# nonl4331/raytracing-rust

Hardware: AMD Instinct MI355X
Metric: Msamples/s on rtweekend1.ssml 1920x1080x1024spp (higher is better)
Workload: dtype f32

## Files before the change

### include/rt_hip.h

```cpp
#ifndef RT_HIP_H
#define RT_HIP_H

#include <stdint.h>

#ifdef __cplusplus
extern "C" {
#endif

#define RT_ABI_VERSION 2u

typedef enum rt_status {
	RT_OK = 0,
	RT_ERR_INVALID_ARGUMENT = -1,
	RT_ERR_NO_DEVICE = -2,
	RT_ERR_HIP = -3,
	RT_ERR_OUT_OF_MEMORY = -4,
	RT_ERR_UNSUPPORTED = -5
} rt_status;

typedef enum rt_texture_type {
	RT_TEX_CHECKERED = 0,
	RT_TEX_SOLID = 1,
	RT_TEX_IMAGE = 2,
	RT_TEX_LERP = 3,
// ... 112 lines not shown
	int32_t render_method;
	uint32_t max_depth;
	uint32_t rr_threshold;
	uint32_t shard_index;
	uint32_t shard_count;
	uint32_t tile_width;
	uint32_t tile_height;
	int32_t output_layout;
	uint32_t sample_split;
	uint32_t reserved0;
} rt_render_opts;

void rt_render_opts_default(rt_render_opts *opts);

typedef struct rt_hit_record {
	float t;
	float point[3];
	float error[3];
	float normal[3];
	float uv[2];
	int32_t has_uv;
	int32_t out;
	uint32_t material;
	uint32_t found;
	uint64_t index;
} rt_hit_record;

typedef struct rt_ray_desc {
	float origin[3];
	float direction[3];
} rt_ray_desc;

typedef struct rt_bvh_node {
	float min[3];
	float max[3];
	int64_t children[2];
	uint64_t primitive_offset;
	uint64_t number_primitives;
} rt_bvh_node;

typedef struct rt_scene rt_scene;

const char *rt_last_error(void);
uint32_t rt_abi_version(void);
int rt_device_count(void);

int rt_camera_new(rt_camera *out, const float origin[3], const float lookat[3], const float vup[3],
                  float fov_degrees, float aspect_ratio, float aperture, float focus_dist);

int rt_scene_create(const rt_scene_desc *desc, int device, rt_scene **out);
#define RT_DEVICE_NONE (-1)
void rt_scene_destroy(rt_scene *scene);

int rt_scene_create_multi(const rt_scene_desc *desc, const int *devices, uint32_t n_devices, rt_scene **out);
int rt_scene_device_count(const rt_scene *scene, uint32_t *n_devices);
typedef enum rt_gather_mode { RT_GATHER_NONE = 0, RT_GATHER_RCCL = 1, RT_GATHER_PEER = 2, RT_GATHER_PEER_STAGED = 3, RT_GATHER_SAME_DEVICE = 4 } rt_gather_mode;
int rt_scene_gather_info(const rt_scene *scene, int *mode, char *note, uint64_t note_capacity);
int rt_rccl_probe(int *usable, char *note, uint64_t note_capacity);
int rt_scene_auto_sample_split(const rt_scene *scene, const rt_render_opts *opts, uint32_t *split);

int rt_scene_counts(const rt_scene *scene, uint64_t *n_nodes, uint64_t *n_primitives, uint64_t *n_lights);
int rt_scene_get_nodes(const rt_scene *scene, rt_bvh_node *out, uint64_t capacity);
int rt_scene_get_primitive_order(const rt_scene *scene, uint64_t *out, uint64_t capacity);
int rt_scene_get_lights(const rt_scene *scene, uint64_t *out, uint64_t capacity);
int rt_scene_wide_info(const rt_scene *scene, uint64_t *n_wide_nodes, uint32_t *root_ref, uint32_t *stack_depth);
int rt_scene_get_wide_nodes(const rt_scene *scene, void *out, uint64_t capacity_nodes);
int rt_scene_get_leaf_boxes(const rt_scene *scene, float *out, uint64_t capacity_slots);
int rt_scene_get_wide_nodes_compact(const rt_scene *scene, void *out, uint64_t capacity_nodes);
int rt_scene_get_leaf_boxes_compact(const rt_scene *scene, float *out, uint64_t capacity_leaves, uint64_t *n_leaves);

typedef struct rt_sky_info {
	uint32_t res_x, res_y;
	uint32_t guide_k;
	uint32_t inv_res_ok;
	float inv_res_x, inv_res_y;
	uint64_t table_bytes;
} rt_sky_info;
int rt_scene_sky_info(const rt_scene *scene, rt_sky_info *info);
int rt_scene_get_sky_tables(const rt_scene *scene, float *row_cdf, uint64_t capacity_rows, float *marginal_cdf, uint64_t capacity_marginal,
                            uint8_t *guide, uint64_t capacity_guide);

int rt_scene_set_traversal(rt_scene *scene, int mode);
typedef enum rt_tuning_key { RT_TUNE_TRAVERSAL = 0, RT_TUNE_FEATURE_SET = 1, RT_TUNE_SCENE_IN_LDS = 2, RT_TUNE_SCHEDULE = 3, RT_TUNE_WALK = 4,
                             RT_TUNE_STACK_CAP = 5, RT_TUNE_EXCHANGE = 6, RT_TUNE_WHOLE_PIXEL_SHARE = 7, RT_TUNE_RADIANCE_GROUPS = 8 } rt_tuning_key;
int rt_scene_set_tuning(rt_scene *scene, int key, int value);
int rt_plan_work_items(const rt_render_opts *opts, uint32_t split, int share, uint64_t resident_waves, uint32_t *whole_claims,
                       uint64_t *n_items);

int rt_render(rt_scene *scene, const rt_camera *camera, const rt_render_opts *opts, float *out_rgb,
              uint64_t *rays_shot);

int rt_render_device(rt_scene *scene, const rt_camera *camera, const rt_render_opts *opts, float *d_out_rgb,
                     uint64_t *d_rays_shot, void *hip_stream);

int rt_render_output_floats(const rt_render_opts *opts, uint64_t *n_floats);
int rt_shard_pixel_order(const rt_render_opts *opts, uint64_t *out, uint64_t capacity);

typedef struct rt_sampler_progress {
	uint64_t samples_completed;
	uint64_t rays_shot;
	const float *current_image;
	uint64_t n_floats;
} rt_sampler_progress;
typedef int (*rt_presentation_update)(void *data, const rt_sampler_progress *progress, uint64_t samples_done);
int rt_sample_image(rt_scene *scene, const rt_camera *camera, const rt_render_opts *opts, uint64_t batch,
                    rt_presentation_update update, void *data);

int rt_last_kernel_ms(rt_scene *scene, float *ms, uint32_t *n_launches);

typedef struct rt_launch_info {
	int32_t method;
	int32_t pruned;
	int32_t fine;
	int32_t sky_in_lds;
	int32_t scene_in_lds;
	int32_t feature_set;
	uint32_t block_threads;
	uint32_t n_blocks;
	uint32_t blocks_per_cu;
	uint32_t waves_per_simd;
	uint32_t lds_bytes;
	uint32_t n_cus;
	uint32_t sample_split;
	uint32_t whole_claims;
	uint64_t n_items;
	char kernel[160];
} rt_launch_info;
int rt_last_launch_info(const rt_scene *scene, rt_launch_info *out);

int rt_output_rgb8(const float *rgb, uint64_t n_values, float gamma, uint8_t *out);
int rt_output_save(const char *filename, const float *rgb, uint32_t width, uint32_t height, float gamma);

int rt_output_rgb8_device(rt_scene *scene, const float *d_rgb, uint64_t n_values, float gamma, uint8_t *d_out, void *hip_stream);
int rt_render_rgb8(rt_scene *scene, const rt_camera *camera, const rt_render_opts *opts, float gamma, uint8_t *out_rgb8,
                   uint64_t *rays_shot);

int rt_check_hit(rt_scene *scene, const rt_ray_desc *rays, uint64_t n_rays, rt_hit_record *out);
int rt_check_hit_index(rt_scene *scene, const rt_ray_desc *rays, const uint64_t *object_index, uint64_t n_rays,
                       rt_hit_record *out);

typedef struct rt_radiance_opts {
	uint64_t seed, sample_begin;
	uint32_t samples_per_ray;
	int32_t  render_method;
	uint32_t max_depth;
	uint32_t rr_threshold;
	uint32_t reserved[2];
} rt_radiance_opts;
int rt_radiance_opts_default(rt_radiance_opts *out);
int rt_radiance(rt_scene *scene, const rt_ray_desc *rays, const uint64_t *streams , uint64_t n_rays,
                const rt_radiance_opts *opts, float *out_rgb);
int rt_radiance_device(rt_scene *scene, const rt_ray_desc *d_rays, const uint64_t *d_streams , uint64_t n_rays,
                       const rt_radiance_opts *opts, float *d_out_rgb, void *hip_stream);

typedef struct rt_aov_buffers {
	float *albedo;
	float *normal;
	float *depth;
	float *coverage;
	uint32_t *primitive;
	uint32_t *material;
} rt_aov_buffers;
int rt_render_aov(rt_scene *scene, const rt_camera *camera, const rt_render_opts *opts, const rt_aov_buffers *host_out);
int rt_render_aov_device(rt_scene *scene, const rt_camera *camera, const rt_render_opts *opts, const rt_aov_buffers *device_out,
                         void *hip_stream);

typedef struct rt_aov_chain_opts {
	uint32_t max_chain;
	float fuzz_limit;
	uint32_t reserved[6];
} rt_aov_chain_opts;
typedef struct rt_aov_chain_buffers {
	rt_aov_buffers aov;
	float *bounces;
} rt_aov_chain_buffers;
int rt_aov_chain_opts_default(rt_aov_chain_opts *out);
int rt_render_aov_chain(rt_scene *scene, const rt_camera *camera, const rt_render_opts *opts, const rt_aov_chain_opts *chain,
                        const rt_aov_chain_buffers *host_out);
int rt_render_aov_chain_device(rt_scene *scene, const rt_camera *camera, const rt_render_opts *opts, const rt_aov_chain_opts *chain,
                               const rt_aov_chain_buffers *device_out, void *hip_stream);

#define RT_MATTE_SLOTS 8u
typedef enum { RT_MATTE_ID_PRIMITIVE = 0, RT_MATTE_ID_MATERIAL = 1 } rt_matte_id_kind;
typedef struct rt_matte_opts {
	int32_t id_kind;
	uint32_t layers;
	uint32_t reserved[6];
} rt_matte_opts;
typedef struct rt_matte_buffers {
	uint32_t *ids;
	float *coverage;
	float *residual;
} rt_matte_buffers;
int rt_matte_opts_default(rt_matte_opts *out);
int rt_render_matte(rt_scene *scene, const rt_camera *camera, const rt_render_opts *opts, const rt_matte_opts *matte,
                    const rt_matte_buffers *host_out);
int rt_render_matte_device(rt_scene *scene, const rt_camera *camera, const rt_render_opts *opts, const rt_matte_opts *matte,
                           const rt_matte_buffers *device_out, void *hip_stream);
int rt_matte_extract(rt_scene *scene, const rt_matte_buffers *host_layers, uint32_t width, uint32_t height, uint32_t layers,
                     const uint32_t *ids, uint64_t n_ids, float *host_out);
int rt_matte_extract_device(rt_scene *scene, const rt_matte_buffers *device_layers, uint32_t width, uint32_t height, uint32_t layers,
                            const uint32_t *d_sorted_ids, uint64_t n_ids, float *d_out, void *hip_stream);

typedef struct rt_ao_opts {
	uint32_t rays_per_pass;
	float radius;
	uint32_t reserved[6];
} rt_ao_opts;
typedef struct rt_ao_buffers {
// ... 226 lines not shown
int rt_selftest_division(float divisor, float *reciprocal, int *exact);

#define RT_SELFTEST_LEAN_CLASSES 9
int rt_selftest_lean(int device, uint64_t n_per_thread, uint64_t seed, uint64_t mismatches[RT_SELFTEST_LEAN_CLASSES]);

enum {
	RT_SHORT_FORM_RCP_REFINED = 0,
	RT_SHORT_FORM_INV_ONE_PAIR = 1,
	RT_SHORT_FORM_INV_TWO_PAIRS = 2,
	RT_SHORT_FORM_SQRT_RAW = 3,
	RT_SHORT_FORM_SQRT_BOTH = 4
};
#define RT_SHORT_FORMS 5
enum { RT_SHORT_SITE_RAY_NEW_PAIR = 0, RT_SHORT_SITE_RAY_NEW_FULL = 1 };
#define RT_SHORT_SITES 2
typedef struct rt_short_form_count {
	uint64_t tested;
	uint64_t mismatches;
	uint32_t first_mismatch;
	uint32_t reserved;
} rt_short_form_count;
typedef struct rt_short_forms_result {
	rt_short_form_count form[RT_SHORT_FORMS];
	uint64_t sqrt_raw_exact, sqrt_raw_high, sqrt_raw_low, sqrt_raw_other;
	uint64_t site_tested;
	uint64_t site_mismatches[RT_SHORT_SITES];
	uint32_t in_use;
	uint32_t reserved;
} rt_short_forms_result;
int rt_selftest_short_forms(int device, const float *operands, uint64_t n_operands, rt_short_forms_result *out);

enum { RT_DIV_FORM_ONE_PAIR = 0, RT_DIV_FORM_TWO_PAIRS = 1 };
#define RT_DIV_FORMS 2
enum { RT_DIV_SITE_FIX = 0, RT_DIV_SITE_DIV3_FIX = 1, RT_DIV_SITE_MIS_LIGHT_TERM = 2, RT_DIV_SITE_ATAN2 = 3 };
#define RT_DIV_SITES 4
typedef struct rt_div_forms_slice {
	const uint32_t *denominators;
	uint64_t n_denominators;
	uint32_t first_denominator;
	uint32_t reserved;
	const int32_t *exponents;
	uint64_t n_exponent_pairs;
} rt_div_forms_slice;
typedef struct rt_div_forms_result {
	uint64_t tested;
	uint64_t mismatches[RT_DIV_FORMS];
	uint32_t first_numerator[RT_DIV_FORMS];
	uint32_t first_denominator[RT_DIV_FORMS];
	uint64_t site_tested;
	uint64_t site_in_domain;
	uint64_t site_mismatches[RT_DIV_SITES];
	uint32_t in_use;
	uint32_t reserved;
} rt_div_forms_result;
int rt_selftest_div_forms(int device, const rt_div_forms_slice *slice, const float *operands, uint64_t n_operand_pairs, rt_div_forms_result *out);
int rt_selftest_sky_pdf_forms(rt_scene *scene, const float *dirs, uint64_t m, float *out_pdf_pair, float *out_pdf_default);

enum { RT_FRAME_FORMS_TESTED = 0, RT_FRAME_FORMS_FRAME_MISMATCHES = 1, RT_FRAME_FORMS_FRAME_SHORT = 2, RT_FRAME_FORMS_FRAME_PLAIN = 3,
       RT_FRAME_FORMS_RAY_MISMATCHES = 4, RT_FRAME_FORMS_RAY_SHORT = 5, RT_FRAME_FORMS_RAY_PLAIN = 6, RT_FRAME_FORMS_IN_USE = 7 };
#define RT_FRAME_FORMS_COUNTS 8
enum { RT_FRAME_FORM_FRAME_SHORT = 0, RT_FRAME_FORM_RAY_NORM_ONE_PAIR = 1 };
int rt_selftest_frame_forms(int device, const float *vectors, uint64_t n_vectors, uint64_t counts[RT_FRAME_FORMS_COUNTS]);

enum { RT_GEN_KEYS_TESTED = 0, RT_GEN_KEYS_STATE_MISMATCHES = 1, RT_GEN_KEYS_DRAW_MISMATCHES = 2, RT_GEN_KEYS_ITEM_STATE_MISMATCHES = 3,
       RT_GEN_KEYS_ITEM_DRAW_MISMATCHES = 4, RT_GEN_KEYS_ZERO_BLOCKS = 5, RT_GEN_KEYS_IN_USE = 6 };
#define RT_GEN_KEYS_COUNTS 7
#define RT_GEN_KEYS_CASE_WORDS 4
enum { RT_GEN_KEYS_FORM_TABLE = 0, RT_GEN_KEYS_FORM_ITEM_PRODUCT = 1 };
int rt_selftest_gen_keys(int device, uint64_t seed, const uint32_t *cases, uint64_t n_cases, uint64_t counts[RT_GEN_KEYS_COUNTS]);
void rt_philox_round_keys(uint64_t seed, uint32_t keys[20]);

enum { RT_PAIR_SHADOW_TESTED = 0, RT_PAIR_SHADOW_MISMATCHES = 1, RT_PAIR_SHADOW_ASKED_MISMATCHES = 2, RT_PAIR_SHADOW_ASKED = 3 };
#define RT_PAIR_SHADOW_COUNTS 4
#define RT_PAIR_SHADOW_CASE_FLOATS 10
int rt_selftest_pair_shadow(int device, const float *cases, uint64_t n_cases, uint64_t counts[RT_PAIR_SHADOW_COUNTS]);
enum { RT_PAIR_SHADOW_WALK_TESTED = 0, RT_PAIR_SHADOW_WALK_MISMATCHES = 1, RT_PAIR_SHADOW_WALK_ASKED = 2, RT_PAIR_SHADOW_WALK_ASKED_BOTH = 3,
       RT_PAIR_SHADOW_WALK_ASKED_WITH_OCCLUDED = 4 };
#define RT_PAIR_SHADOW_WALK_COUNTS 5
#define RT_PAIR_SHADOW_WALK_CASE_FLOATS 16
int rt_selftest_pair_shadow_walk(int device, const float *cases, uint64_t n_cases, uint64_t counts[RT_PAIR_SHADOW_WALK_COUNTS]);

int rt_selftest_pair_primary(rt_scene *scene, const float origin[3], uint32_t *valid, uint64_t *mismatches);

int rt_selftest_sky(rt_scene *scene, int tables_in_lds, uint64_t seed, uint64_t n, float *out_dirs, float *out_pdf_of_sample,
                    const float *dirs, uint64_t m, float *out_pdf);

#ifdef __cplusplus
}
#endif
#endif
```

### raytracing-rust_amd/abi.py

```python
import ctypes as C

RT_ABI_VERSION = 2
RT_GATHER_NONE, RT_GATHER_RCCL, RT_GATHER_PEER, RT_GATHER_PEER_STAGED, RT_GATHER_SAME_DEVICE = 0, 1, 2, 3, 4

RT_OK = 0
RT_ERR_INVALID_ARGUMENT = -1
RT_ERR_NO_DEVICE = -2
RT_ERR_HIP = -3
RT_ERR_OUT_OF_MEMORY = -4
RT_ERR_UNSUPPORTED = -5

RT_TEX_CHECKERED, RT_TEX_SOLID, RT_TEX_IMAGE, RT_TEX_LERP, RT_TEX_PERLIN = range(5)
RT_MAT_EMIT, RT_MAT_LAMBERTIAN, RT_MAT_TROWBRIDGE_REITZ, RT_MAT_REFLECT, RT_MAT_REFRACT = range(5)
RT_PRIM_SPHERE, RT_PRIM_TRIANGLE, RT_PRIM_MESH_TRIANGLE = range(3)
RT_SPLIT_SAH, RT_SPLIT_MIDDLE, RT_SPLIT_EQUAL_COUNTS = range(3)
RT_METHOD_NAIVE, RT_METHOD_MIS = range(2)
RT_LAYOUT_FRAME, RT_LAYOUT_SHARD = range(2)
RT_TUNE_TRAVERSAL, RT_TUNE_FEATURE_SET, RT_TUNE_SCENE_IN_LDS, RT_TUNE_SCHEDULE, RT_TUNE_WALK, RT_TUNE_STACK_CAP, RT_TUNE_EXCHANGE, RT_TUNE_WHOLE_PIXEL_SHARE = range(8)
RT_TUNE_RADIANCE_GROUPS = 8

NO_INDEX = 0xFFFFFFFFFFFFFFFF
RT_DEVICE_NONE = -1

f32x3 = C.c_float * 3


class TextureDesc(C.Structure):
    _fields_ = [
        ("type", C.c_int32),
        ("colour_one", f32x3),
        ("colour_two", f32x3),
        ("image_rgb", C.POINTER(C.c_float)),
        ("image_width", C.c_uint32),
        ("image_height", C.c_uint32),
        ("perlin_ran_vecs", C.POINTER(C.c_float)),
        ("perlin_perm", C.POINTER(C.c_uint32)),
    ]


class MaterialDesc(C.Structure):
    _fields_ = [
        ("type", C.c_int32),
        ("texture", C.c_uint32),
        ("param", C.c_float),
        ("ior", f32x3),
        ("metallic", C.c_float),
    ]


class _Sphere(C.Structure):
    _fields_ = [("centre", f32x3), ("radius", C.c_float)]


class _MeshTriangle(C.Structure):
    _fields_ = [("mesh", C.c_uint32), ("point_indices", C.c_uint32 * 3), ("normal_indices", C.c_uint32 * 3)]


class _Triangle(C.Structure):
    _fields_ = [("data", C.c_uint64)]


class _PrimUnion(C.Union):
    _fields_ = [("sphere", _Sphere), ("mesh_triangle", _MeshTriangle), ("triangle", _Triangle)]


class PrimitiveDesc(C.Structure):
    _fields_ = [("type", C.c_int32), ("material", C.c_uint32), ("u", _PrimUnion)]


class TriangleData(C.Structure):
    _fields_ = [("points", C.c_float * 9), ("normals", C.c_float * 9)]


class MeshDesc(C.Structure):
    _fields_ = [
        ("vertices", C.POINTER(C.c_float)),
        ("n_vertices", C.c_uint64),
        ("normals", C.POINTER(C.c_float)),
        ("n_normals", C.c_uint64),
    ]


class SkyDesc(C.Structure):
    _fields_ = [
        ("texture", C.c_uint32),
        ("material", C.c_uint32),
        ("sampler_res_x", C.c_uint32),
        ("sampler_res_y", C.c_uint32),
    ]


class SceneDesc(C.Structure):
    _fields_ = [
        ("abi_version", C.c_uint32),
        ("n_textures", C.c_uint32),
        ("textures", C.POINTER(TextureDesc)),
        ("n_materials", C.c_uint32),
        ("n_meshes", C.c_uint32),
        ("materials", C.POINTER(MaterialDesc)),
        ("meshes", C.POINTER(MeshDesc)),
        ("n_primitives", C.c_uint64),
        ("primitives", C.POINTER(PrimitiveDesc)),
# ... 3 lines not shown
        ("split_type", C.c_int32),
    ]


class Camera(C.Structure):
    _fields_ = [("origin", f32x3), ("lower_left", f32x3), ("horizontal", f32x3), ("vertical", f32x3)]


class RenderOpts(C.Structure):
    _fields_ = [
        ("width", C.c_uint64),
        ("height", C.c_uint64),
        ("samples_per_pixel", C.c_uint64),
        ("sample_begin", C.c_uint64),
        ("seed", C.c_uint64),
        ("render_method", C.c_int32),
        ("max_depth", C.c_uint32),
        ("rr_threshold", C.c_uint32),
        ("shard_index", C.c_uint32),
        ("shard_count", C.c_uint32),
        ("tile_width", C.c_uint32),
        ("tile_height", C.c_uint32),
        ("output_layout", C.c_int32),
        ("sample_split", C.c_uint32),
        ("reserved0", C.c_uint32),
    ]


class HitRecord(C.Structure):
    _fields_ = [
        ("t", C.c_float),
        ("point", f32x3),
        ("error", f32x3),
        ("normal", f32x3),
        ("uv", C.c_float * 2),
        ("has_uv", C.c_int32),
        ("out", C.c_int32),
        ("material", C.c_uint32),
        ("found", C.c_uint32),
        ("index", C.c_uint64),
    ]


class RayDesc(C.Structure):
    _fields_ = [("origin", f32x3), ("direction", f32x3)]


class BvhNode(C.Structure):
    _fields_ = [
        ("min", f32x3),
        ("max", f32x3),
        ("children", C.c_int64 * 2),
        ("primitive_offset", C.c_uint64),
        ("number_primitives", C.c_uint64),
    ]


class SamplerProgressC(C.Structure):
    _fields_ = [
        ("samples_completed", C.c_uint64),
        ("rays_shot", C.c_uint64),
        ("current_image", C.POINTER(C.c_float)),
        ("n_floats", C.c_uint64),
    ]


class LaunchInfo(C.Structure):
    _fields_ = [
        ("method", C.c_int32),
        ("pruned", C.c_int32),
        ("fine", C.c_int32),
        ("sky_in_lds", C.c_int32),
        ("scene_in_lds", C.c_int32),
        ("feature_set", C.c_int32),
        ("block_threads", C.c_uint32),
        ("n_blocks", C.c_uint32),
        ("blocks_per_cu", C.c_uint32),
        ("waves_per_simd", C.c_uint32),
        ("lds_bytes", C.c_uint32),
        ("n_cus", C.c_uint32),
        ("sample_split", C.c_uint32),
        ("whole_claims", C.c_uint32),
        ("n_items", C.c_uint64),
        ("kernel", C.c_char * 160),
    ]


class SkyInfo(C.Structure):
    _fields_ = [
        ("res_x", C.c_uint32),
        ("res_y", C.c_uint32),
        ("guide_k", C.c_uint32),
        ("inv_res_ok", C.c_uint32),
        ("inv_res_x", C.c_float),
        ("inv_res_y", C.c_float),
        ("table_bytes", C.c_uint64),
    ]


class AovBuffers(C.Structure):
    _fields_ = [
        ("albedo", C.POINTER(C.c_float)),
        ("normal", C.POINTER(C.c_float)),
        ("depth", C.POINTER(C.c_float)),
        ("coverage", C.POINTER(C.c_float)),
        ("primitive", C.POINTER(C.c_uint32)),
        ("material", C.POINTER(C.c_uint32)),
    ]


AOV_SHAPES = {"albedo": "hw3", "normal": "hw3", "depth": "hw", "coverage": "hw", "primitive": "hw", "material": "hw"}
AOV_CHANNELS = tuple(AOV_SHAPES)


class AovChainOpts(C.Structure):
    _fields_ = [
        ("max_chain", C.c_uint32),
        ("fuzz_limit", C.c_float),
        ("reserved", C.c_uint32 * 6),
    ]


class AovChainBuffers(C.Structure):
    _fields_ = [
        ("aov", AovBuffers),
        ("bounces", C.POINTER(C.c_float)),
    ]


AOV_CHAIN_SHAPES = {"aov": AOV_SHAPES, "bounces": "hw"}
AOV_CHAIN_CHANNELS = AOV_CHANNELS + ("bounces",)
AOV_CHAIN_MAX_CHAIN = 64


RT_MATTE_SLOTS = 8
RT_MATTE_ID_PRIMITIVE, RT_MATTE_ID_MATERIAL = range(2)
MATTE_ID_KINDS = {"primitive": RT_MATTE_ID_PRIMITIVE, "material": RT_MATTE_ID_MATERIAL}
MATTE_MAX_IDS = 1 << 20


class MatteOpts(C.Structure):
    _fields_ = [
        ("id_kind", C.c_int32),
        ("layers", C.c_uint32),
        ("reserved", C.c_uint32 * 6),
    ]


class MatteBuffers(C.Structure):
    _fields_ = [
        ("ids", C.POINTER(C.c_uint32)),
        ("coverage", C.POINTER(C.c_float)),
        ("residual", C.POINTER(C.c_float)),
    ]


MATTE_SHAPES = {"ids": "lhw", "coverage": "lhw", "residual": "hw"}
MATTE_BUFFERS = tuple(MATTE_SHAPES)


AO_MAX_RAYS = 64


class AoOpts(C.Structure):
    _fields_ = [
        ("rays_per_pass", C.c_uint32),
        ("radius", C.c_float),
# ... 337 lines not shown
    "rt_aov_chain_buffers": (AovChainBuffers, 56),
    "rt_matte_opts": (MatteOpts, 32),
    "rt_matte_buffers": (MatteBuffers, 24),
    "rt_ao_opts": (AoOpts, 32),
    "rt_ao_buffers": (AoBuffers, 16),
    "rt_radiance_opts": (RadianceOpts, 40),
    "rt_noise_opts": (NoiseOpts, 32),
    "rt_noise_summary": (NoiseSummary, 16),
    "rt_noise_buffers": (NoiseBuffers, 40),
    "rt_noise_result": (NoiseResult, 40),
    "rt_adaptive_result": (AdaptiveResult, 40),
    "rt_robust_opts": (RobustOpts, 32),
    "rt_robust_buffers": (RobustBuffers, 40),
    "rt_denoise_opts": (DenoiseOpts, 48),
    "rt_denoise_inputs": (DenoiseInputs, 40),
    "rt_temporal_opts": (TemporalOpts, 96),
    "rt_temporal_inputs": (TemporalInputs, 32),
    "rt_display_opts": (DisplayOpts, 104),
    "rt_display_state": (DisplayState, 16),
    "rt_bloom_opts": (BloomOpts, 64),
    "rt_dof_opts": (DofOpts, 64),
    "rt_upscale_opts": (UpscaleOpts, 56),
    "rt_upscale_inputs": (UpscaleInputs, 56),
    "rt_short_form_count": (ShortFormCount, 24),
    "rt_short_forms_result": (ShortFormsResult, 184),
    "rt_div_forms_slice": (DivFormsSlice, 40),
    "rt_div_forms_result": (DivFormsResult, 96),
}

EXPORTED_SYMBOLS = [
    "rt_last_error",
    "rt_abi_version",
    "rt_device_count",
    "rt_render_opts_default",
    "rt_camera_new",
    "rt_scene_create",
    "rt_scene_create_multi",
    "rt_scene_device_count",
    "rt_scene_destroy",
    "rt_scene_counts",
    "rt_scene_get_nodes",
    "rt_scene_get_primitive_order",
    "rt_scene_get_lights",
    "rt_scene_wide_info",
    "rt_scene_get_wide_nodes",
    "rt_scene_get_leaf_boxes",
    "rt_scene_get_wide_nodes_compact",
    "rt_scene_auto_sample_split",
    "rt_scene_gather_info",
    "rt_rccl_probe",
    "rt_selftest_division",
    "rt_scene_get_leaf_boxes_compact",
    "rt_scene_sky_info",
    "rt_scene_get_sky_tables",
    "rt_scene_set_traversal",
    "rt_scene_set_tuning",
    "rt_render",
    "rt_sample_image",
    "rt_render_device",
    "rt_render_output_floats",
    "rt_shard_pixel_order",
    "rt_plan_work_items",
    "rt_last_kernel_ms",
    "rt_last_launch_info",
    "rt_output_rgb8",
    "rt_output_save",
    "rt_output_rgb8_device",
    "rt_render_rgb8",
    "rt_check_hit",
    "rt_check_hit_index",
    "rt_radiance_opts_default",
    "rt_radiance",
    "rt_radiance_device",
    "rt_selftest_lean",
    "rt_selftest_short_forms",
    "rt_selftest_div_forms",
    "rt_selftest_sky_pdf_forms",
    "rt_selftest_frame_forms",
    "rt_selftest_gen_keys",
    "rt_philox_round_keys",
    "rt_selftest_pair_shadow",
    "rt_selftest_pair_shadow_walk",
    "rt_selftest_pair_primary",
    "rt_selftest_sky",
    "rt_render_aov",
    "rt_render_aov_device",
    "rt_aov_chain_opts_default",
    "rt_render_aov_chain",
    "rt_render_aov_chain_device",
    "rt_matte_opts_default",
    "rt_render_matte",
    "rt_render_matte_device",
    "rt_matte_extract",
    "rt_matte_extract_device",
    "rt_ao_opts_default",
    "rt_render_ao",
    "rt_render_ao_device",
    "rt_denoise_opts_default",
    "rt_denoise_workspace_bytes",
    "rt_denoise",
    "rt_denoise_device",
    "rt_render_denoised",
    "rt_noise_opts_default",
    "rt_render_noise",
    "rt_render_noise_device",
    "rt_noise_tiles",
    "rt_noise_tiles_device",
    "rt_render_converged",
    "rt_render_denoised_split",
    "rt_render_adaptive",
    "rt_render_tiles",
    "rt_render_tiles_device",
    "rt_noise_select_tiles",
    "rt_noise_select_tiles_device",
    "rt_robust_opts_default",
    "rt_render_robust",
    "rt_render_robust_device",
    "rt_robust_combine",
    "rt_robust_combine_device",
    "rt_render_denoised_robust",
    "rt_temporal_opts_default",
    "rt_temporal_history_bytes",
    "rt_temporal_workspace_bytes",
    "rt_denoise_temporal_device",
    "rt_denoise_temporal",
    "rt_denoise_temporal_reset",
    "rt_display_opts_default",
    "rt_display_workspace_bytes",
    "rt_display_output_bytes",
    "rt_display_device",
    "rt_display",
    "rt_display_reset",
    "rt_bloom_opts_default",
    "rt_bloom_workspace_bytes",
    "rt_bloom_device",
    "rt_bloom",
    "rt_dof_opts_default",
    "rt_dof_opts_from_camera",
    "rt_dof_workspace_bytes",
    "rt_dof_device",
    "rt_dof",
    "rt_render_dof",
    "rt_upscale_opts_default",
    "rt_upscale_device",
    "rt_upscale",
    "rt_render_upscaled",
]


def channels(table, struct):
    out = {}
    for name, shape in table.items():
        if isinstance(shape, dict):
            out.update(channels(shape, getattr(struct, name)))
        else:
            out[name] = (struct, dict(struct._fields_)[name]._type_, shape)
    return out


def default_aov_chain_opts(max_chain=8, fuzz_limit=0.0):
    o = AovChainOpts()
    o.max_chain, o.fuzz_limit = max_chain, fuzz_limit
    return o


def default_matte_opts(id_kind=RT_MATTE_ID_MATERIAL, layers=4):
# ... 46 lines not shown
```

### raytracing-rust_amd/csrc/rt_api.cpp

```cpp
#include <hip/hip_runtime.h>

#include <cstdio>
#include <cstdlib>
#include <algorithm>
#include <cmath>
#include <cstring>
#include <string>
#include <vector>

#include "../../include/rt_hip.h"
#include "../../include/rt_detmath.h"
#include <dlfcn.h>
#include "rt_api_internal.h"
#include "rt_render.h"

using namespace rt;

thread_local std::string g_error;

constexpr uint32_t kFineAboveTriangles = 4096;
constexpr uint32_t kFineAboveSpheres = 32768;

struct RcclApi {
	void *lib = nullptr;
// ... 567 lines not shown
		return fail(RT_ERR_INVALID_ARGUMENT, "null argument");
	*mode = s->peers.empty() ? RT_GATHER_NONE : s->gather_mode;
	if (note && note_capacity) {
		std::strncpy(note, s->gather_note.c_str(), (size_t)note_capacity - 1);
		note[note_capacity - 1] = 0;
	}
	return RT_OK;
}

int rt_scene_device_count(const rt_scene *s, uint32_t *n_devices)
{
	if (!s || !n_devices)
		return fail(RT_ERR_INVALID_ARGUMENT, "null argument");
	*n_devices = s->device == RT_DEVICE_NONE ? 0u : (uint32_t)(1 + s->peers.size());
	return RT_OK;
}

int rt_scene_set_traversal(rt_scene *s, int mode)
{
	if (!s || mode < -1 || mode > 1)
		return fail(RT_ERR_INVALID_ARGUMENT, "bad arguments");
	s->traversal_mode = mode;
	for (rt_scene *m : s->peers)
		m->traversal_mode = mode;
	return RT_OK;
}

static int set_tuning_one(rt_scene *s, int key, int value);
int rt_scene_set_tuning(rt_scene *s, int key, int value)
{
	if (!s)
		return fail(RT_ERR_INVALID_ARGUMENT, "null scene");
	const int rc = set_tuning_one(s, key, value);
	for (rt_scene *m : s->peers)
		if (rc == RT_OK) {
			(void)set_tuning_one(m, key, value);
		}
	return rc;
}
static int set_tuning_one(rt_scene *s, int key, int value)
{
	switch (key) {
	case RT_TUNE_TRAVERSAL:
		return rt_scene_set_traversal(s, value);
	case RT_TUNE_FEATURE_SET:
		if (value < s->min_feature_set || value > 2)
			return fail(RT_ERR_INVALID_ARGUMENT, "feature set must be between the scene's own and 2");
		s->feature_set = value;
		s->feature_set_forced = true;
		return RT_OK;
	case RT_TUNE_SCHEDULE:
		if (value < -1 || value > 1)
			return fail(RT_ERR_INVALID_ARGUMENT, "schedule must be -1, 0 or 1");
		s->schedule_mode = value;
		return RT_OK;
	case RT_TUNE_SCENE_IN_LDS:
		s->scene_lds_allowed = value != 0;
		return RT_OK;
	case RT_TUNE_STACK_CAP:
		if (value < 0 || value > 96)
			return fail(RT_ERR_INVALID_ARGUMENT, "stack cap must be 0 (automatic) or 1..96 entries");
		s->stack_cap_override = (uint32_t)value;
		return RT_OK;
	case RT_TUNE_EXCHANGE:
		if (value < 0 || value > 1)
			return fail(RT_ERR_INVALID_ARGUMENT, "exchange must be 0 (off) or 1 (on where the kernel has it)");
		s->exchange_mode = value;
		return RT_OK;
	case RT_TUNE_WHOLE_PIXEL_SHARE:
		if (value < -1 || value > 16)
			return fail(RT_ERR_INVALID_ARGUMENT, "whole-pixel share must be -1 (automatic) or 0..16 (sixteenths of a shard's tiles)");
		s->whole_share = value;
		return RT_OK;
	case RT_TUNE_WALK:
		if (value < 0 || value > 1)
			return fail(RT_ERR_INVALID_ARGUMENT, "walk must be 0 (automatic) or 1 (two-child walk for every ray)");
		s->dev.narrow_only = (uint32_t)value;
		return RT_OK;
	case RT_TUNE_RADIANCE_GROUPS:
		if (value < 0 || value > 65536)
			return fail(RT_ERR_INVALID_ARGUMENT, "radiance groups must be 0 (automatic) or 1..65536 workgroups");
		s->radiance_groups = (uint32_t)value;
		return RT_OK;
	default:
		return fail(RT_ERR_INVALID_ARGUMENT, "unknown tuning key");
	}
}

int rt_scene_counts(const rt_scene *s, uint64_t *n_nodes, uint64_t *n_primitives, uint64_t *n_lights)
{
	if (!s)
		return fail(RT_ERR_INVALID_ARGUMENT, "null scene");
	if (n_nodes) *n_nodes = s->host.nodes.size();
	if (n_primitives) *n_primitives = s->host.primitive_order.size();
	if (n_lights) *n_lights = s->host.lights.size();
	return RT_OK;
}
int rt_scene_get_nodes(const rt_scene *s, rt_bvh_node *out, uint64_t capacity)
{
	if (!s || !out || capacity < s->host.nodes.size())
		return fail(RT_ERR_INVALID_ARGUMENT, "bad arguments");
	for (size_t i = 0; i < s->host.nodes.size(); ++i) {
		const HostNode &n = s->host.nodes[i];
		std::memcpy(out[i].min, n.min, 12);
		std::memcpy(out[i].max, n.max, 12);
		out[i].children[0] = n.child[0];
		out[i].children[1] = n.child[1];
		out[i].primitive_offset = n.primitive_offset;
		out[i].number_primitives = n.number_primitives;
	}
	return RT_OK;
}
int rt_scene_get_primitive_order(const rt_scene *s, uint64_t *out, uint64_t capacity)
{
	if (!s || !out || capacity < s->host.primitive_order.size())
		return fail(RT_ERR_INVALID_ARGUMENT, "bad arguments");
	std::memcpy(out, s->host.primitive_order.data(), s->host.primitive_order.size() * sizeof(uint64_t));
	return RT_OK;
}
int rt_scene_wide_info(const rt_scene *s, uint64_t *n_wide_nodes, uint32_t *root_ref, uint32_t *stack_depth)
{
	if (!s)
		return fail(RT_ERR_INVALID_ARGUMENT, "null scene");
	if (n_wide_nodes) *n_wide_nodes = s->host.dev_nodes4.size();
	if (root_ref) *root_ref = s->host.root4_ref;
	if (stack_depth) *stack_depth = s->host.stack_depth;
	return RT_OK;
}
int rt_scene_get_wide_nodes(const rt_scene *s, void *out, uint64_t capacity_nodes)
{
	if (!s || !out || capacity_nodes < s->host.dev_nodes4.size())
		return fail(RT_ERR_INVALID_ARGUMENT, "bad arguments");
	std::memcpy(out, s->host.dev_nodes4.data(), s->host.dev_nodes4.size() * sizeof(DevNodeQ4));
	return RT_OK;
}
int rt_scene_get_leaf_boxes(const rt_scene *s, float *out, uint64_t capacity_slots)
{
	if (!s || !out || capacity_slots < s->host.leaf_box.size())
		return fail(RT_ERR_INVALID_ARGUMENT, "bad arguments");
	std::memcpy(out, s->host.leaf_box.data(), s->host.leaf_box.size() * sizeof(DevLeafBox));
	return RT_OK;
}
int rt_scene_get_wide_nodes_compact(const rt_scene *s, void *out, uint64_t capacity_nodes)
{
	if (!s || !out || capacity_nodes < s->host.dev_nodes4c.size())
		return fail(RT_ERR_INVALID_ARGUMENT, "bad arguments");
	std::memcpy(out, s->host.dev_nodes4c.data(), s->host.dev_nodes4c.size() * sizeof(DevNodeQ4));
	return RT_OK;
}
int rt_scene_get_leaf_boxes_compact(const rt_scene *s, float *out, uint64_t capacity_leaves, uint64_t *n_leaves)
{
	if (!s)
		return fail(RT_ERR_INVALID_ARGUMENT, "null scene");
	if (n_leaves)
		*n_leaves = s->host.leaf_box_c.size();
	if (!out)
		return n_leaves ? RT_OK : fail(RT_ERR_INVALID_ARGUMENT, "bad arguments");
	if (capacity_leaves < s->host.leaf_box_c.size())
		return fail(RT_ERR_INVALID_ARGUMENT, "bad arguments");
	std::memcpy(out, s->host.leaf_box_c.data(), s->host.leaf_box_c.size() * sizeof(DevLeafBox));
	return RT_OK;
}
int rt_scene_sky_info(const rt_scene *s, rt_sky_info *info)
{
	if (!s || !info)
		return fail(RT_ERR_INVALID_ARGUMENT, "null argument");
// ... 127 lines not shown
	return RT_OK;
}

static void fill_tiling(DevRenderParams &P, const rt_render_opts *o, const ShardGeometry &g)
{
	P.width = (uint32_t)o->width;
	P.height = (uint32_t)o->height;
	P.shard_index = o->shard_index;
	P.shard_count = o->shard_count;
	P.tile_w = g.tile_w;
	P.tile_h = g.tile_h;
	P.tiles_x = g.tiles_x;
	P.tiles_y = g.tiles_y;
	P.n_work = (uint32_t)g.n_work;
}

static uint32_t tiled_order_log2(const rt_render_opts *o, const ShardGeometry &g, uint32_t split)
{
	if (g.tile_w * g.tile_h == 64u && (g.tile_w & (g.tile_w - 1u)) == 0u && o->width < 65536u && o->height < 65536u &&
	    (split & (split - 1u)) == 0u && split <= 64u)
		for (uint32_t lw = 0; lw < 7u; ++lw)
			for (uint32_t ls = 0; ls < 7u; ++ls)
				if ((1u << lw) == g.tile_w && (1u << ls) == split)
					return lw | (ls << 8);
	return 0xFFFFFFFFu;
}

struct RenderLaunchPlan {
	DevRenderParams P;
	DevScene dev;
	bool prune, fine, sky_lds, scene_lds, xchg;
	int feature_set, blocks_per_cu;
	uint32_t block_threads, n_blocks;
	size_t lds_bytes;
	uint32_t split;
};

static int plan_render_launch(const rt_scene *s, const rt_render_opts *o, const ShardGeometry &g, RenderLaunchPlan *plan)
{
	DevRenderParams P;
	std::memset(&P, 0, sizeof P);
	fill_tiling(P, o, g);
	P.spp = (uint32_t)o->samples_per_pixel;
	P.sample_begin_lo = (uint32_t)o->sample_begin;
	P.sample_begin_hi = (uint32_t)(o->sample_begin >> 32);
	P.seed_lo = (uint32_t)o->seed;
	P.seed_hi = (uint32_t)(o->seed >> 32);
	P.max_depth = o->max_depth;
	P.rr_threshold = o->rr_threshold;
	uint32_t split = o->sample_split;
	if (split == 0u)
		split = auto_sample_split(s->n_cus, o->width * o->height, o->samples_per_pixel, o->shard_count);
	{
		float rw = 0.0f, rh = 0.0f;
		const bool sized = o->width <= (1u << 24) && o->height <= (1u << 24);
		const bool ok_w = sized && verified_reciprocal((float)(o->width - 1), &rw), ok_h = sized && verified_reciprocal((float)(o->height - 1), &rh);
		const bool ok = ok_w && ok_h;
		P.w1h1_ok = ok ? 1u : 0u;
		P.inv_w1 = rw;
		P.inv_h1 = rh;
	}
	P.tile_log2_w = tiled_order_log2(o, g, split);
	if (split > o->samples_per_pixel)
		return fail(RT_ERR_INVALID_ARGUMENT, "sample_split larger than samples_per_pixel");
	if (g.n_work * split >= (1ull << 32))
		return fail(RT_ERR_UNSUPPORTED, "pixels x sample_split exceeds 2^32 work items");
	P.sample_split = split;
	P.shard_layout = o->output_layout == RT_LAYOUT_SHARD ? 1 : 0;

	bool prune = scene_prunes(s);
	const bool fine = s->dev.nodes4 != nullptr &&
	                  (s->schedule_mode == -1 ? (prune && s->dev.n_prims > (s->dev.has_triangles ? kFineAboveTriangles : kFineAboveSpheres))
	                                          : s->schedule_mode == 1);
	if (fine)
		prune = true;
	P.prune = prune ? 1 : 0;

	const bool samplable = (s->dev.sky.res_x | s->dev.sky.res_y) != 0u;
	const size_t sky_bytes = sky_table_bytes(s->dev.sky.res_x, s->dev.sky.res_y, s->dev.sky.guide_k);
	const bool scene_lds = !fine && s->dev.blob_bytes != 0u && s->scene_lds_allowed;
	P.scene_in_lds = scene_lds ? 1u : 0u;
	bool sky_lds = false;
	const int feature_set =
	    (s->feature_set == 0 && s->pair_tree && !s->feature_set_forced && !prune && !fine && s->exchange_mode != 1) ? 3 : s->feature_set;
	bool xchg = s->exchange_mode == 1 && render_exchange_available(o->render_method, prune, fine, feature_set);
	const bool xchg_fine = xchg && fine;
	uint32_t block_threads = render_block_threads(feature_set, fine, xchg_fine);
	const size_t fine_pool_bytes = xchg_fine ? render_exchange_fine_lds_bytes(block_threads / 64u) : 0;
	DevScene dev = s->dev;
	const bool walks_wide = prune && dev.nodes4 != nullptr && dev.narrow_only == 0u;
	uint32_t stack_need = (fine || walks_wide) ? dev.stack_depth : s->stack_depth_narrow;
	if (!fine && walks_wide &&
	    render_lds_bytes(dev, false, scene_lds, render_block_threads(feature_set, false, false) / 64u, stack_need) > s->max_lds) {
		dev.narrow_only = 1u;
		stack_need = s->stack_depth_narrow;
	}
	uint32_t stack_cap = stack_need;
	if (fine) {
		const uint32_t blocks_wanted = std::max(1u, render_waves_per_simd(feature_set, true) * 256u / block_threads);
		const size_t share = s->max_lds / blocks_wanted;
		const uint32_t fit = (uint32_t)((share > fine_pool_bytes ? share - fine_pool_bytes : 0) / ((block_threads / 64u) * 64u * 4u));
		stack_cap = std::min(stack_cap, std::max(8u, fit));
	}
	if (fine && s->stack_cap_override != 0u)
		stack_cap = std::min(stack_need, s->stack_cap_override);
	P.stack_cap = stack_cap;
	P.stack_ovf_depth = stack_need - stack_cap;
	const bool sky_lds_possible = samplable && o->render_method == RT_METHOD_MIS && sky_bytes <= kSkyLdsLimit;
	struct Sizing { uint32_t block; int blocks_per_cu; bool sky; size_t lds; };
	auto size_launch = [&](uint32_t block, Sizing &z) -> hipError_t {
		z.block = block;
		z.sky = false;
		z.blocks_per_cu = 0;
		z.lds = render_lds_bytes(dev, false, scene_lds, block / 64u, stack_cap) + fine_pool_bytes;
		if (z.lds > s->max_lds)
			return hipSuccess;
		hipError_t e = render_occupancy(o->render_method, prune, fine, false, feature_set, z.lds, &z.blocks_per_cu, xchg_fine, block);
		if (e != hipSuccess)
			return e;
		if (sky_lds_possible) {
			const size_t lds_with = render_lds_bytes(dev, true, scene_lds, block / 64u, stack_cap) + fine_pool_bytes;
			int blocks_with = 0;
			if (lds_with <= s->max_lds &&
			    render_occupancy(o->render_method, prune, fine, true, feature_set, lds_with, &blocks_with, xchg_fine, block) == hipSuccess &&
			    blocks_with >= z.blocks_per_cu && blocks_with >= 1) {
				z.sky = true;
				z.lds = lds_with;
				z.blocks_per_cu = blocks_with;
			}
		}
		return hipSuccess;
	};
	Sizing Z;
	HIP_TRY(size_launch(block_threads, Z));
	if (Z.lds > s->max_lds)
		return fail(RT_ERR_UNSUPPORTED, "traversal stacks exceed the LDS of one CU");
	if (!fine && !xchg) {
		for (uint32_t cand = block_threads + 256u; cand <= render_max_block_threads(feature_set, fine, false); cand += 256u) {
			Sizing C;
			if (size_launch(cand, C) != hipSuccess || C.blocks_per_cu < 1)
				continue;
			const uint32_t waves_c = (uint32_t)C.blocks_per_cu * C.block, waves_z = (uint32_t)Z.blocks_per_cu * Z.block;
			if (waves_c > waves_z || (waves_c == waves_z && C.sky && !Z.sky))
				Z = C;
		}
		block_threads = Z.block;
	}
	size_t lds_bytes = Z.lds;
	int blocks_per_cu = Z.blocks_per_cu;
	sky_lds = Z.sky;
	P.sky_in_lds = sky_lds ? 1u : 0u;
	if (blocks_per_cu < 1)
		return fail(RT_ERR_HIP, "render kernel does not fit on a CU");
	P.xchg_slots = 0;
	if (xchg && !fine) {
		int blocks_plain = 0;
		if (render_occupancy(o->render_method, prune, fine, sky_lds, feature_set, lds_bytes, &blocks_plain, true) != hipSuccess || blocks_plain < 1) {
			xchg = false;
		} else {
			const int target = std::min(blocks_per_cu, blocks_plain);
			const size_t share = s->max_lds / (size_t)target;
			uint32_t slots = render_exchange_max_slots();
			while (slots >= 16u && lds_bytes + render_exchange_lds_bytes(slots) > share)
				slots -= 4u;
			int blocks_x = 0;
			if (slots >= 16u &&
			    render_occupancy(o->render_method, prune, fine, sky_lds, feature_set, lds_bytes + render_exchange_lds_bytes(slots), &blocks_x, true) == hipSuccess &&
// ... 236 lines not shown
	}
	if (d_rays_shot) {
		for (uint32_t m = 0; m < n; ++m) {
			if (n_floats[m] == 0) {
				HIP_TRY(hipMemsetAsync(head->d_gather_rays + m, 0, sizeof(unsigned long long), stream));
			} else if (members[m]->device == head->device) {
				if (m > 0 && head->gather_mode == RT_GATHER_RCCL)
					HIP_TRY(hipStreamWaitEvent(stream, members[m]->ev_shard, 0));
				HIP_TRY(hipMemcpyAsync(head->d_gather_rays + m, members[m]->d_member_rays, sizeof(unsigned long long), hipMemcpyDeviceToDevice, stream));
			} else {
				if (head->gather_mode == RT_GATHER_RCCL)
					HIP_TRY(hipStreamWaitEvent(stream, members[m]->ev_shard, 0));
				HIP_TRY(hipMemcpyPeerAsync(head->d_gather_rays + m, head->device, members[m]->d_member_rays, members[m]->device, sizeof(unsigned long long), stream));
			}
		}
		HIP_TRY(launch_sum_u64(stream, head->d_gather_rays, n, reinterpret_cast<unsigned long long *>(d_rays_shot)));
	}
	if (!capturing) {
		HIP_TRY(hipEventRecord(head->ev_gathered, stream));
		head->gathered_once = true;
	}
	return RT_OK;
}

int rt_render_device(rt_scene *s, const rt_camera *camera, const rt_render_opts *o, float *d_out_rgb, uint64_t *d_rays_shot,
                     void *hip_stream)
{
	if (!s || !camera || !o || !d_out_rgb)
		return fail(RT_ERR_INVALID_ARGUMENT, "null argument");
	if (!s->peers.empty() && !s->member_call) {
		if (s->device == RT_DEVICE_NONE)
			return fail(RT_ERR_NO_DEVICE, "host-only scene");
		return render_device_multi(s, camera, o, d_out_rgb, d_rays_shot, static_cast<hipStream_t>(hip_stream));
	}
	ShardGeometry g;
	int rc = shard_geometry(o, g);
	if (rc != RT_OK)
		return rc;
	if (s->device == RT_DEVICE_NONE)
		return fail(RT_ERR_NO_DEVICE, "host-only scene (RT_DEVICE_NONE): rendering needs a GPU, there is no CPU fallback");
	if (o->render_method != RT_METHOD_NAIVE && o->render_method != RT_METHOD_MIS)
		return fail(RT_ERR_INVALID_ARGUMENT, "unknown render method");
	if (o->samples_per_pixel == 0 || o->samples_per_pixel >= (1ull << 32))
		return fail(RT_ERR_INVALID_ARGUMENT, "samples_per_pixel must be in [1, 2^32)");
	if (o->output_layout != RT_LAYOUT_FRAME && o->output_layout != RT_LAYOUT_SHARD)
		return fail(RT_ERR_INVALID_ARGUMENT, "unknown output layout");
	HIP_TRY(hipSetDevice(s->device));
	hipStream_t stream = static_cast<hipStream_t>(hip_stream);
	if (g.n_work == 0) {
		HIP_TRY(launch_reset(stream, s->d_work_counter, reinterpret_cast<unsigned long long *>(d_rays_shot), d_out_rgb,
		                     o->output_layout == RT_LAYOUT_FRAME ? (size_t)(o->width * o->height * 3) : 0));
		s->timed = false;
		return RT_OK;
	}

	RenderLaunchPlan plan;
	rc = plan_render_launch(s, o, g, &plan);
	if (rc != RT_OK)
		return rc;
	const DevRenderParams &P = plan.P;
	float *render_target = d_out_rgb;
	if (plan.split > 1u) {
		const size_t need = (size_t)g.n_work * plan.split * 3;
		rc = grow_device_buffer(s->d_partial, s->partial_floats, need);
		if (rc != RT_OK)
			return rc;
		render_target = s->d_partial;
	}
	if (P.stack_ovf_depth != 0u) {
		const size_t need = (size_t)plan.n_blocks * plan.block_threads * P.stack_ovf_depth;
		rc = grow_device_buffer(s->d_stack_ovf, s->stack_ovf_words, need);
		if (rc != RT_OK)
			return rc;
	}
	{
		size_t zero_floats = 0;
		if (o->output_layout == RT_LAYOUT_FRAME && o->shard_count > 1)
			zero_floats = (size_t)(o->width * o->height * 3);
		if (o->output_layout == RT_LAYOUT_SHARD)
			zero_floats = (size_t)(g.n_work * 3);
		HIP_TRY(launch_reset(stream, s->d_work_counter, reinterpret_cast<unsigned long long *>(d_rays_shot), d_out_rgb, zero_floats));
	}
	fill_launch_info(plan, o, s->n_cus, &s->last_launch);
	const DevCamera cam = dev_camera(camera);
	DevPairPrimary primary{};
	if (plan.feature_set == 3)
		pair_primary_terms(s->pair, plan.dev.root_min, plan.dev.root_max, v3(cam.origin[0], cam.origin[1], cam.origin[2]), primary);
	HIP_TRY(hipEventRecord(s->ev_start, stream));
	HIP_TRY(launch_render(o->render_method, plan.prune, plan.fine, plan.sky_lds, plan.feature_set, plan.n_blocks, plan.lds_bytes, stream, plan.dev, cam, P,
	                      render_target, reinterpret_cast<unsigned long long *>(d_rays_shot), s->d_work_counter, s->d_stack_ovf, plan.xchg,
	                      plan.feature_set == 3 ? &s->pair : nullptr, plan.feature_set == 3 ? &primary : nullptr, plan.block_threads));
	HIP_TRY(hipEventRecord(s->ev_stop, stream));
	if (plan.split > 1u)
		HIP_TRY(launch_combine(stream, P, s->d_partial, d_out_rgb));
	s->timed = true;
	s->n_launches = 1;
	return RT_OK;
}

int rt_render(rt_scene *s, const rt_camera *camera, const rt_render_opts *o, float *out_rgb, uint64_t *rays_shot)
{
	if (!s || !camera || !o)
		return fail(RT_ERR_INVALID_ARGUMENT, "null argument");
	if (int rc = need_device(s); rc != RT_OK)
		return rc;
	uint64_t n_floats = 0;
	int rc = rt_render_output_floats(o, &n_floats);
	if (rc != RT_OK)
		return rc;
	if (n_floats == 0) {
		if (rays_shot)
			*rays_shot = 0;
		return RT_OK;
	}
	if (!out_rgb)
		return fail(RT_ERR_INVALID_ARGUMENT, "null argument");
	HIP_TRY(hipSetDevice(s->device));
	rc = ensure_frame_buffers(s, n_floats, false);
	if (rc != RT_OK)
		return rc;
	float *d_out = s->d_prog[0];
	rc = rt_render_device(s, camera, o, d_out, reinterpret_cast<uint64_t *>(s->d_rays), s->stream);
	if (rc != RT_OK)
		return rc;
	Staging st{s};
	st.download(out_rgb, d_out, n_floats * sizeof(float));
	st.download(rays_shot, s->d_rays, sizeof(uint64_t));
	return st.finish("render");
}

int rt_output_rgb8_device(rt_scene *s, const float *d_rgb, uint64_t n_values, float gamma, uint8_t *d_out, void *hip_stream)
{
	if (!s || !d_rgb || !d_out)
		return fail(RT_ERR_INVALID_ARGUMENT, "null argument");
	if (s->device == RT_DEVICE_NONE)
		return fail(RT_ERR_NO_DEVICE, "host-only scene (RT_DEVICE_NONE): this call needs a GPU (rt_output_rgb8 is the host-side conversion)");
	if (n_values == 0)
		return RT_OK;
	HIP_TRY(hipSetDevice(s->device));
	HIP_TRY(launch_quantise(static_cast<hipStream_t>(hip_stream), d_rgb, (size_t)n_values, 1.0f / gamma, d_out));
	return RT_OK;
}

int rt_render_rgb8(rt_scene *s, const rt_camera *camera, const rt_render_opts *o, float gamma, uint8_t *out_rgb8, uint64_t *rays_shot)
{
	if (!s || !camera || !o)
		return fail(RT_ERR_INVALID_ARGUMENT, "null argument");
	if (int rc = need_device(s); rc != RT_OK)
		return rc;
	uint64_t n_values = 0;
	int rc = rt_render_output_floats(o, &n_values);
	if (rc != RT_OK)
		return rc;
	if (n_values == 0) {
		if (rays_shot)
			*rays_shot = 0;
		return RT_OK;
	}
	if (!out_rgb8)
		return fail(RT_ERR_INVALID_ARGUMENT, "null argument");
	HIP_TRY(hipSetDevice(s->device));
	rc = ensure_frame_buffers(s, n_values, false);
	if (rc != RT_OK)
		return rc;
	rc = grow_device_buffer(s->d_rgb8, s->d_rgb8_bytes, (size_t)n_values);
	if (rc != RT_OK)
		return rc;
	float *d_frame = s->d_prog[0];
	rc = rt_render_device(s, camera, o, d_frame, reinterpret_cast<uint64_t *>(s->d_rays), s->stream);
	if (rc != RT_OK)
		return rc;
	Staging st{s};
	st.e = launch_quantise(s->stream, d_frame, (size_t)n_values, 1.0f / gamma, s->d_rgb8);
	st.download(out_rgb8, s->d_rgb8, n_values);
// ... 116 lines not shown
```

### raytracing-rust_amd/csrc/rt_api_internal.h

```cpp
#pragma once
#include <hip/hip_runtime.h>

#include <cstdint>
#include <cstring>
#include <string>
#include <vector>

#include "../../include/rt_hip.h"
#include "rt_build.h"
#include "rt_layout.h"
#include "rt_types.h"

extern thread_local std::string g_error;

inline int fail(int code, const std::string &msg)
{
	g_error = msg;
	return code;
}
inline int hip_fail(hipError_t e, const char *what)
{
	g_error = std::string(what) + ": " + hipGetErrorString(e);
	return e == hipErrorOutOfMemory ? RT_ERR_OUT_OF_MEMORY : RT_ERR_HIP;
}
#define HIP_TRY(expr)                       \
	do {                                    \
		hipError_t e_ = (expr);             \
		if (e_ != hipSuccess)               \
			return hip_fail(e_, #expr);     \
	} while (0)
#define RT_TRY(expr)            \
	do {                        \
		const int rc_ = (expr); \
		if (rc_ != RT_OK)       \
			return rc_;         \
	} while (0)

constexpr uint32_t kPruneAbove = 100;

constexpr int kWholeShareDefault = -1;

struct rt_scene {
	int device = 0;
	rt::HostScene host;
	rt::DevScene dev{};
	std::vector<void *> allocations;
	hipStream_t stream = nullptr;
	uint32_t *d_work_counter = nullptr;
	unsigned long long *d_rays = nullptr;
	hipEvent_t ev_start = nullptr, ev_stop = nullptr;
	bool timed = false;
	uint32_t n_launches = 0;
	int n_cus = 0;
	int traversal_mode = -1;
	int schedule_mode = -1;
	int feature_set = 2;
	int min_feature_set = 0;
	bool pair_tree = false, feature_set_forced = false;
	rt::DevPairScene pair{};
	bool scene_lds_allowed = true;
	float *d_partial = nullptr;
	size_t partial_floats = 0;
	float *d_prog[2] = {nullptr, nullptr};
	float *h_prog[2] = {nullptr, nullptr};
	unsigned long long *d_prog_rays = nullptr;
	unsigned long long *h_prog_rays = nullptr;
	size_t d_prog_floats[2] = {0, 0}, h_prog_floats[2] = {0, 0};
	hipStream_t copy_stream = nullptr;
	hipEvent_t ev_batch[2] = {nullptr, nullptr}, ev_copy[2] = {nullptr, nullptr};
	size_t max_lds = 65536;
	rt_launch_info last_launch{};
	uint32_t stack_cap_override = 0;
	int exchange_mode = 0;
	int whole_share = kWholeShareDefault;
	uint32_t radiance_groups = 0;
	uint32_t stack_depth_narrow = 2;
	uint32_t *d_stack_ovf = nullptr;
	size_t stack_ovf_words = 0;
	uint8_t *d_rgb8 = nullptr;
	size_t d_rgb8_bytes = 0;
	std::vector<rt_scene *> peers;
	bool member_call = false;
	float *d_shard = nullptr;
	size_t shard_floats = 0;
	unsigned long long *d_member_rays = nullptr;
	hipEvent_t ev_shard = nullptr;
	hipEvent_t ev_begin = nullptr;
	float *d_gather = nullptr;
	size_t gather_floats = 0;
	unsigned long long *d_gather_rays = nullptr;
	void *nccl_comms = nullptr;
	int gather_mode = 0;
	std::string gather_note;
	hipEvent_t ev_gathered = nullptr;
	bool gathered_once = false;
	uint32_t *d_prim_desc = nullptr;
	char *d_denoise = nullptr;
	size_t d_denoise_bytes = 0;
	char *d_temporal = nullptr;
	uint32_t temporal_w = 0, temporal_h = 0;
	int temporal_cur = -1;
	rt_camera temporal_prev{};
	char *d_display = nullptr;
	size_t d_display_bytes = 0;
	uint32_t display_w = 0, display_h = 0;
	bool display_has_state = false;
	char *d_noise = nullptr;
	size_t d_noise_bytes = 0;
	char *d_bloom = nullptr;
	size_t d_bloom_bytes = 0;
	char *d_dof = nullptr;
	size_t d_dof_bytes = 0;
};

uint32_t auto_sample_split(int n_cus, uint64_t frame_pixels, uint64_t spp, uint32_t n_sharers);
struct WorkItems { uint64_t whole_claims, n_items; };
WorkItems plan_work_items(uint64_t tiles, uint64_t tile_pixels, uint32_t split, bool tiled, int share, uint64_t resident_waves);

constexpr size_t kSkyLdsLimit = 96 * 1024;
inline size_t sky_table_bytes(uint32_t res_x, uint32_t res_y, uint32_t guide_k)
{
	if ((res_x | res_y) == 0u)
		return 0;
	return ((size_t)res_y * (res_x + 1u) + res_y + 1u) * 4 + (size_t)(res_y + 1u) * guide_k;
}

inline bool scene_prunes(const rt_scene *s)
{
	return s->traversal_mode == -1 ? s->dev.n_prims > kPruneAbove : s->traversal_mode == 1;
}

inline int four_wave_traversal(const rt_scene *s, bool *prune, rt::DevScene *dev)
{
	*prune = scene_prunes(s);
	*dev = s->dev;
	const bool walks_wide = *prune && dev->nodes4 != nullptr && dev->narrow_only == 0u;
	if (!walks_wide || rt::four_wave_stack_lds_bytes(*dev) > s->max_lds) {
		if (walks_wide)
			dev->narrow_only = 1u;
		dev->stack_depth = s->stack_depth_narrow;
	}
	if (rt::four_wave_stack_lds_bytes(*dev) > s->max_lds)
		return fail(RT_ERR_UNSUPPORTED, "traversal stacks exceed the LDS of one CU");
	return RT_OK;
}

inline uint32_t path_lane_groups(const rt_scene *s, size_t lds_bytes, uint32_t waves, uint64_t wanted)
{
	const uint64_t by_lds = std::max<uint64_t>(1, (160u * 1024u) / std::max<size_t>(1, lds_bytes));
	const uint64_t resident = (uint64_t)std::max(1, s->n_cus) * std::min<uint64_t>(waves, by_lds);
	uint64_t groups = std::min<uint64_t>(wanted, resident);
	if (s->radiance_groups != 0u)
		groups = std::min<uint64_t>(groups, s->radiance_groups);
	return (uint32_t)std::max<uint64_t>(groups, 1);
}


struct TileGrid { uint32_t tiles_x; uint64_t count; };
inline TileGrid tile_grid(uint64_t w, uint64_t h)
{
	const uint64_t across = (w + 7) / 8, down = (h + 7) / 8;
	return TileGrid{(uint32_t)across, across * down};
}

struct FrameTiling { uint32_t tile_w, tile_h, tiles_x, tiles_y; uint64_t n_work; };
inline FrameTiling frame_tiling(const rt_render_opts *o)
{
	FrameTiling t;
	t.tile_w = o->tile_width ? o->tile_width : 8;
	t.tile_h = o->tile_height ? o->tile_height : 8;
	t.tiles_x = (uint32_t)((o->width + t.tile_w - 1) / t.tile_w);
	t.tiles_y = (uint32_t)((o->height + t.tile_h - 1) / t.tile_h);
	t.n_work = (uint64_t)t.tiles_x * t.tiles_y * t.tile_w * t.tile_h;
	return t;
}

inline rt::DevCamera dev_camera(const rt_camera *camera)
{
	rt::DevCamera cam;
	std::memcpy(cam.origin, camera->origin, 12);
	std::memcpy(cam.lower_left, camera->lower_left, 12);
	std::memcpy(cam.horizontal, camera->horizontal, 12);
	std::memcpy(cam.vertical, camera->vertical, 12);
	return cam;
}

template <class T> static int upload(rt_scene *s, const T *src, size_t count, const T **dst)
{
	void *p = nullptr;
	const size_t bytes = (count ? count : 1) * sizeof(T);
	HIP_TRY(hipMalloc(&p, bytes));
	s->allocations.push_back(p);
	if (count)
		HIP_TRY(hipMemcpy(p, src, count * sizeof(T), hipMemcpyHostToDevice));
	*dst = static_cast<const T *>(p);
	return RT_OK;
}

inline bool ranges_overlap(const void *a, uint64_t a_bytes, const void *b, uint64_t b_bytes)
{
	if (!a || !b)
		return false;
	const uintptr_t x = reinterpret_cast<uintptr_t>(a), y = reinterpret_cast<uintptr_t>(b);
	return x < y + b_bytes && y < x + a_bytes;
}


inline int need_device(const rt_scene *s)
{
	if (s->device == RT_DEVICE_NONE)
		return fail(RT_ERR_NO_DEVICE, "host-only scene (RT_DEVICE_NONE): this call needs a GPU, there is no CPU fallback");
	return RT_OK;
}

inline int frame_sides(const char *stage, uint64_t w, uint64_t h, uint64_t min_side)
{
	if (w >= min_side && h >= min_side)
		return RT_OK;
	return fail(RT_ERR_INVALID_ARGUMENT, stage + ("width and height must be >= " + std::to_string(min_side)) +
	                                         (min_side >= 2 ? " (u and v divide by W-1 and H-1)" : ""));
}

inline int frame_pixels(const char *stage, uint64_t w, uint64_t h, uint64_t min_side, uint64_t *n)
{
	if (const int rc = frame_sides(stage, w, h, min_side); rc != RT_OK)
		return rc;
	if (w > (1ull << 31) || h > (1ull << 31) || w * h > (1ull << 31))
		return fail(RT_ERR_UNSUPPORTED, std::string(stage) + "more than 2^31 pixels");
	*n = w * h;
	return RT_OK;
}

inline int check_disjoint(const char *message, const void *const buf[], const uint64_t bytes[], int n_written, int n_total)
{
	for (int a = 0; a < n_written; ++a)
		for (int b = 0; b < n_total; ++b)
			if (a != b && ranges_overlap(buf[a], bytes[a], buf[b], bytes[b]))
				return fail(RT_ERR_INVALID_ARGUMENT, message);
	return RT_OK;
}

template <class T> static int grow_device_buffer(T *&p, size_t &count, size_t need)
{
	if (need <= count)
		return RT_OK;
	if (p)
		(void)hipFree(p);
	p = nullptr;
	count = 0;
	HIP_TRY(hipMalloc(reinterpret_cast<void **>(&p), need * sizeof(T)));
	count = need;
	return RT_OK;
}

static int grow_device_buffer(char *&p, size_t &bytes, rt::Layout &L)
{
	if (L.overflowed)
		return fail(RT_ERR_UNSUPPORTED, "internal: a buffer layout of more parts than rt::Layout holds");
	const int rc = grow_device_buffer(p, bytes, (size_t)L.total());
// ... 30 lines not shown
```

### raytracing-rust_amd/csrc/rt_api_query.cpp

```cpp
#include <hip/hip_runtime.h>

#include <algorithm>
#include <cstring>
#include <vector>

#include "../../include/rt_hip.h"
#include "rt_api_internal.h"
#include "rt_query.h"
#include "rt_radiance.h"
#include "rt_selftest.h"
#include "rt_gen_keys.h"

using namespace rt;

#ifdef RT_STATS
extern "C" int rt_debug_trace_queue(rt_scene *s, const rt_ray_desc *rays, uint64_t n, int waves, uint32_t cap, float *out_t, uint32_t *out_prim,
                                    float *ms, unsigned long long *node_steps)
{
	if (!s || !rays || !out_t || !out_prim || n == 0 || n >= (1ull << 31) || s->device == RT_DEVICE_NONE || s->dev.nodes4 == nullptr)
		return fail(RT_ERR_INVALID_ARGUMENT, "bad arguments (or no wide tree)");
	HIP_TRY(hipSetDevice(s->device));
	cap = std::min(std::max(cap, 1u), s->dev.stack_depth);
	const uint32_t ovf_depth = s->dev.stack_depth - cap;
	const uint32_t n_blocks = (uint32_t)s->n_cus * (uint32_t)waves;
// ... 361 lines not shown
	for (int k = 0; k < RT_DIV_SITES; ++k)
		out->site_mismatches[k] = host[kDivCountSiteBad + k];
	out->in_use = div_forms_in_use();
	return RT_OK;
}

int rt_selftest_sky_pdf_forms(rt_scene *s, const float *dirs, uint64_t m, float *out_pdf_pair, float *out_pdf_default)
{
	if (!s || !dirs || !out_pdf_pair || !out_pdf_default || m == 0 || m > (1ull << 24))
		return fail(RT_ERR_INVALID_ARGUMENT, "bad arguments (1 to 2^24 directions)");
	if ((s->host.sky.sampler_res_x | s->host.sky.sampler_res_y) == 0u)
		return fail(RT_ERR_INVALID_ARGUMENT, "the sky is not samplable (sampler_res 0 x 0)");
	if (int rc = need_device(s); rc != RT_OK)
		return rc;
	Layout L;
	const auto p_dirs = L.add<float>(3 * m), p_pair = L.add<float>(m), p_default = L.add<float>(m);
	RT_TRY(sky_buffer(s, L));
	Staging st{s};
	st.put(L, p_dirs, dirs);
	if (st.ok())
		st.e = launch_sky_pdf_forms(s->stream, s->dev, L.at(p_dirs), m, L.at(p_pair), L.at(p_default));
	st.get(out_pdf_pair, L, p_pair);
	st.get(out_pdf_default, L, p_default);
	return sky_finish(st, L, "selftest_sky_pdf_forms");
}

int rt_selftest_pair_shadow(int device, const float *cases, uint64_t n_cases, uint64_t counts[RT_PAIR_SHADOW_COUNTS])
{
	return run_case_table<RT_PAIR_SHADOW_COUNTS>(device, cases, n_cases, RT_PAIR_SHADOW_CASE_FLOATS * sizeof(float), counts, "selftest_pair_shadow",
	                                             launch_pair_shadow);
}
int rt_selftest_pair_shadow_walk(int device, const float *cases, uint64_t n_cases, uint64_t counts[RT_PAIR_SHADOW_WALK_COUNTS])
{
	return run_case_table<RT_PAIR_SHADOW_WALK_COUNTS>(device, cases, n_cases, RT_PAIR_SHADOW_WALK_CASE_FLOATS * sizeof(float), counts,
	                                                  "selftest_pair_shadow_walk", launch_pair_shadow_walk);
}
int rt_selftest_frame_forms(int device, const float *vectors, uint64_t n_vectors, uint64_t counts[RT_FRAME_FORMS_COUNTS])
{
	RT_TRY(run_case_table<RT_FRAME_FORMS_COUNTS>(device, vectors, n_vectors, 3 * sizeof(float), counts, "selftest_frame_forms", launch_frame_forms));
	counts[RT_FRAME_FORMS_IN_USE] = frame_forms_in_use();
	return RT_OK;
}
int rt_selftest_gen_keys(int device, uint64_t seed, const uint32_t *cases, uint64_t n_cases, uint64_t counts[RT_GEN_KEYS_COUNTS])
{
	RT_TRY(run_case_table<RT_GEN_KEYS_COUNTS>(device, cases, n_cases, RT_GEN_KEYS_CASE_WORDS * sizeof(uint32_t), counts, "selftest_gen_keys",
	                                          [seed](hipStream_t stream, const uint32_t *d_cases, uint64_t n, unsigned long long *d_counts) {
		                                          return launch_gen_keys(stream, seed, d_cases, n, d_counts);
	                                          }));
	counts[RT_GEN_KEYS_IN_USE] = gen_keys_in_use();
	return RT_OK;
}

void rt_philox_round_keys(uint64_t seed, uint32_t keys[20])
{
	if (!keys)
		return;
	DevGenKeys K;
	philox_round_keys(seed, K);
	for (int r = 0; r < 10; ++r) {
		keys[2 * r] = K.key[r][0];
		keys[2 * r + 1] = K.key[r][1];
	}
}

int rt_selftest_pair_primary(rt_scene *s, const float origin[3], uint32_t *valid, uint64_t *mismatches)
{
	if (!s || !origin || !valid || !mismatches)
		return fail(RT_ERR_INVALID_ARGUMENT, "null argument");
	if (int rc = need_device(s); rc != RT_OK)
		return rc;
	if (!s->pair_tree)
		return fail(RT_ERR_UNSUPPORTED, "not a scene the two-sphere kernels take");
	DevPairPrimary host{};
	pair_primary_terms(s->pair, s->dev.root_min, s->dev.root_max, v3(origin[0], origin[1], origin[2]), host);
	unsigned long long bad = 0;
	RT_TRY(run_cases(s->device, nullptr, 0, &bad, 1, "selftest_pair_primary", [&](unsigned long long *d, void *) {
		return launch_selftest_pair_primary(nullptr, s->pair, s->dev.root_min, s->dev.root_max, origin, host, d);
	}));
	*valid = host.valid;
	*mismatches = bad;
	return RT_OK;
}

}
```

### raytracing-rust_amd/csrc/rt_intersect.h

```cpp
#pragma once

#include "rt_types.h"
#include "rt_lean.h"

namespace rt {

struct Ray {
	V3 o, d, inv, shear;
};

template <class F> __device__ __forceinline__ Ray ray_new(V3 origin, V3 direction)
{
	Ray r;
	r.o = origin;
#if defined(__HIP_DEVICE_COMPILE__) && !defined(RT_NO_LEAN)
	const float m2 = dot(direction, direction);
	const float smallest = fminf(fminf(fabsf(direction.x), fabsf(direction.y)), fabsf(direction.z));
	if (__builtin_expect(smallest >= 0x1p-60f && m2 >= 0x1p-40f && m2 <= 0x1p40f, 1)) {
		direction = lean_div3_for<lean_ray_norm_short(F::pair)>(direction, lean_sqrt(m2));
		r.d = direction;
		r.inv = v3(lean_inv_for<F::pair>(direction.x), lean_inv_for<F::pair>(direction.y), lean_inv_for<F::pair>(direction.z));
		if (F::tri) {
			const float ax = fabsf(direction.x), ay = fabsf(direction.y), az = fabsf(direction.z);
			const bool swap = (ax > ay && ax > az) || (ay > az);
			const float sx = swap ? direction.z : direction.x;
			const float sz = swap ? direction.x : direction.z;
			const float rz = lean_rcp_refined(sz);
			r.shear = v3(lean_div_core(-sx, sz, rz), lean_div_core(-direction.y, sz, rz), lean_div_core(1.0f, sz, rz));
		} else {
			r.shear = v3s(0.0f);
		}
		return r;
	}
#endif
	direction = direction / mag(direction);
	r.d = direction;
	r.inv = v3(1.0f / direction.x, 1.0f / direction.y, 1.0f / direction.z);
	if (F::tri) {
		const float ax = fabsf(direction.x), ay = fabsf(direction.y), az = fabsf(direction.z);
		const bool swap = (ax > ay && ax > az) || (ay > az);
		const float sx = swap ? direction.z : direction.x;
		const float sz = swap ? direction.x : direction.z;
		r.shear = v3(-sx / sz, -direction.y / sz, 1.0f / sz);
	} else {
		r.shear = v3s(0.0f);
	}
	return r;
}
__device__ __forceinline__ bool ray_swaps_xz(const Ray &r)
{
	const float ax = fabsf(r.d.x), ay = fabsf(r.d.y), az = fabsf(r.d.z);
	return (ax > ay && ax > az) || (ay > az);
}

template <class D> __device__ __forceinline__ bool aabb_slabs(const D &delta, const V3 &inv, float &tmin_out)
{
	constexpr float widen = 1.0f + 2.0f * gamma_n(3);
	float t1 = delta(0, false) * inv.x;
	float t2 = delta(0, true) * inv.x;
	if (t1 > t2) { const float s = t1; t1 = t2; t2 = s; }
	t2 *= widen;
	float tmin = fmin_(t1, t2);
	float tmax = fmax_(t1, t2);

	t1 = delta(1, false) * inv.y;
	t2 = delta(1, true) * inv.y;
	if (t1 > t2) { const float s = t1; t1 = t2; t2 = s; }
	t2 *= widen;
	tmin = fmax_(tmin, fmin_(t1, t2));
	tmax = fmin_(tmax, fmax_(t1, t2));

	t1 = delta(2, false) * inv.z;
	t2 = delta(2, true) * inv.z;
	if (t1 > t2) { const float s = t1; t1 = t2; t2 = s; }
	t2 *= widen;
	tmin = fmax_(tmin, fmin_(t1, t2));
	tmax = fmin_(tmax, fmax_(t1, t2));

	tmin_out = tmin;
	return tmax > fmax_(tmin, 0.0f);
}
__device__ __forceinline__ bool aabb_does_int(const float bmin[3], const float bmax[3], const Ray &r, float &tmin_out)
{
	const float o[3] = {r.o.x, r.o.y, r.o.z};
	return aabb_slabs([&](int axis, bool upper) { return (upper ? bmax[axis] : bmin[axis]) - o[axis]; }, r.inv, tmin_out);
}
__device__ __forceinline__ bool aabb_does_int_from(const float dmin[3], const float dmax[3], const V3 &inv, float &tmin_out)
{
	return aabb_slabs([&](int axis, bool upper) { return upper ? dmax[axis] : dmin[axis]; }, inv, tmin_out);
}

__device__ __forceinline__ float sqrt_from_(float x)
{
// ... 806 lines not shown
```

### raytracing-rust_amd/csrc/rt_render.h

```cpp
#pragma once
#include <hip/hip_runtime.h>
#include "rt_types.h"

namespace rt {
size_t render_lds_bytes(const DevScene &S, bool sky_lds, bool scene_lds, uint32_t waves_per_block, uint32_t stack_cap);
uint32_t render_waves_per_simd(int feature_set, bool fine);
uint32_t render_block_threads(int feature_set, bool fine, bool xchg = false);
uint32_t render_max_block_threads(int feature_set, bool fine, bool xchg);
hipError_t render_occupancy(int method, bool prune, bool fine, bool sky_lds, int feature_set, size_t lds_bytes, int *blocks_per_cu, bool xchg,
                            uint32_t block_threads = 0);
bool render_exchange_available(int method, bool prune, bool fine, int feature_set);
size_t render_exchange_lds_bytes(uint32_t slots);
uint32_t render_exchange_max_slots();
size_t render_exchange_fine_lds_bytes(uint32_t waves_per_block);

hipError_t launch_reset(hipStream_t stream, uint32_t *work_counter, unsigned long long *rays_shot, float *out, size_t n_out_floats);
hipError_t launch_render(int method, bool prune, bool fine, bool sky_lds, int feature_set, uint32_t n_blocks, size_t lds_bytes, hipStream_t stream,
                         const DevScene &S, const DevCamera &cam, const DevRenderParams &P, float *out,
                         unsigned long long *rays_shot, uint32_t *work_counter, uint32_t *stack_ovf, bool xchg, const DevPairScene *pair,
                         const DevPairPrimary *primary, uint32_t block_threads = 0);
hipError_t launch_combine(hipStream_t stream, const DevRenderParams &P, const float *partial, float *out);
hipError_t launch_scatter_shard(hipStream_t stream, const DevRenderParams &P, const float *shard, float *frame);
hipError_t launch_sum_u64(hipStream_t stream, const unsigned long long *parts, uint32_t n, unsigned long long *out);
hipError_t launch_quantise(hipStream_t stream, const float *rgb, size_t n_values, float inv_gamma, uint8_t *out);
}
```

### raytracing-rust_amd/csrc/rt_render.hip

```cpp
#include "rt_shade.h"
#include "rt_gen_keys.h"
#include "rt_render.h"

namespace rt {

enum : int {
	PH_GEN = 0,
	PH_NODE = 1,
	PH_LEAF = 2,
	PH_SHADE = 3,
	PH_LIGHT = 4,
	PH_SCATTER = 5,
	PH_NARROW = 6,
	PH_COUNT = 7,
	PH_NEED_PIXEL = 7,
	PH_DONE = 8,
	PH_WALK = 9
};

#ifndef RT_PQ_SPLIT
#define RT_PQ_SPLIT 1
#endif
#ifndef RT_LIGHT_PHASE_THRESHOLD
#define RT_LIGHT_PHASE_THRESHOLD 48
#endif
constexpr uint32_t kLightPhaseThreshold = RT_LIGHT_PHASE_THRESHOLD;
#ifndef RT_STARVE_LIMIT
#define RT_STARVE_LIMIT 128
#endif
constexpr uint32_t kStarveLimit = RT_STARVE_LIMIT;
constexpr uint32_t kClaim = 64;
constexpr uint32_t kWholePixel = 64u;
constexpr uint32_t kWholeClaim = 1u << 31;
#ifndef RT_ACQUIRE_BATCH
#define RT_ACQUIRE_BATCH 1
#endif
constexpr uint32_t kAcquireBatch = RT_ACQUIRE_BATCH;
#ifndef RT_FULL_WAVES
#define RT_FULL_WAVES 5
#endif
#ifndef RT_FULL_FINE_WAVES
#define RT_FULL_FINE_WAVES 4
#endif
#ifndef RT_SIMPLE_FINE_WAVES
#define RT_SIMPLE_FINE_WAVES 4
#endif
#ifndef RT_SIMPLE_COARSE_WAVES
#define RT_SIMPLE_COARSE_WAVES 5
#endif
#ifndef RT_SIMPLE_COARSE_BLOCK
#define RT_SIMPLE_COARSE_BLOCK 256
#endif
#ifndef RT_SPHERES_BLOCK
#define RT_SPHERES_BLOCK 512
#endif
#ifndef RT_FUSE_REGIONS
#define RT_FUSE_REGIONS(spheres_only) true
#endif
#ifndef RT_BODY_ALWAYS
#define RT_BODY_ALWAYS(spheres_only) true
#endif
#ifndef RT_SPHERES_MAX_BLOCK
#define RT_SPHERES_MAX_BLOCK 768
#endif
#ifndef RT_PAIR_WAVES
#define RT_PAIR_WAVES 6
#endif
#ifndef RT_SPHERES_WAVES
#define RT_SPHERES_WAVES 4
#endif
#ifndef RT_SPHERES_COARSE_WAVES
#define RT_SPHERES_COARSE_WAVES 6
#endif

__device__ __forceinline__ float power_heuristic(float pdf_a, float pdf_b)
{
	const float a_sq = pdf_a * pdf_a;
	return a_sq / (a_sq + pdf_b * pdf_b);
}

__device__ __forceinline__ bool work_to_pixel(const DevRenderParams &P, uint32_t w, uint32_t &x, uint32_t &y)
{
	const uint32_t tile_pixels = P.tile_w * P.tile_h;
	const uint32_t k = w / tile_pixels;
	const uint32_t in = w - k * tile_pixels;
	const uint32_t tile = P.shard_index + k * P.shard_count;
	const uint32_t ty = tile / P.tiles_x;
	const uint32_t tx = tile - ty * P.tiles_x;
	x = tx * P.tile_w + in % P.tile_w;
	y = ty * P.tile_h + in / P.tile_w;
	return x < P.width && y < P.height;
}

template <class F, bool FINE = false, bool XCHG = false> struct KernelShape {
	static constexpr bool spheres_only = !(F::tri || F::lights || F::cmat || F::ctex);
	static constexpr bool simple = !spheres_only && !(F::cmat || F::ctex);
	static constexpr int waves_per_simd = (F::cmat || F::ctex) ? (FINE ? RT_FULL_FINE_WAVES : (XCHG ? 3 : RT_FULL_WAVES))
	                                      : (F::pair ? RT_PAIR_WAVES : (spheres_only ? ((FINE || XCHG) ? RT_SPHERES_WAVES : RT_SPHERES_COARSE_WAVES)
	                                                                                 : (FINE ? RT_SIMPLE_FINE_WAVES : (XCHG ? 4 : RT_SIMPLE_COARSE_WAVES))));
	static constexpr int block = (FINE && XCHG) ? 512 : (spheres_only ? RT_SPHERES_BLOCK : ((simple && !FINE) ? RT_SIMPLE_COARSE_BLOCK : 256));
	static constexpr int max_block = ((spheres_only || simple) && !FINE && !XCHG && block == 512) ? RT_SPHERES_MAX_BLOCK : block;
};

#ifdef RT_STATS
#define RT_SECTION(k) do { const unsigned long long now_ = wall_clock64(); st_sect[(k)] += now_ - st_mark; st_mark = now_; } while (0)
#else
#define RT_SECTION(k) do { } while (0)
#endif
#ifdef RT_STATS
__device__ unsigned long long g_stats[64];
__device__ unsigned long long g_hist[4][65];
#endif

constexpr uint32_t kXchgBStride = 44, kXchgPStride = 12;
constexpr uint32_t kXchgMaxSlots = 64;
constexpr uint32_t kXchgMinLanes = 4;
constexpr uint32_t kXchgRecWords = 60;
constexpr uint32_t kXchgFineSlots = 64;
constexpr uint32_t kXchgFineHdr = 8 + 2 * 64;
#ifndef RT_XCHG_SHADERS
#define RT_XCHG_SHADERS 1
#endif
constexpr uint32_t kXchgShaderWaves = RT_XCHG_SHADERS;
enum : uint32_t { XS_EMPTY = 0, XS_FULL = 1, XS_BUSY = 2 };

struct RenderArgs {
	DevScene S;
	DevCamera cam;
	DevRenderParams P;
	float *out;
	unsigned long long *rays_shot;
	uint32_t *work_counter;
	uint32_t *stack_ovf;
	DevPairScene pair;
	DevPairPrimary primary;
	DevGenKeys gen_keys;
};
#if defined(__HIP_DEVICE_COMPILE__)
typedef const __attribute__((address_space(4))) RenderArgs *KArgs;
#else
typedef const RenderArgs *KArgs;
#endif

template <int METHOD, bool PRUNE, bool FINE, bool SKY_LDS, class F, bool XCHG = false>
__global__ __launch_bounds__((KernelShape<F, FINE, XCHG>::max_block), (KernelShape<F, FINE, XCHG>::waves_per_simd)) void render_kernel(const RenderArgs args_by_value)
{
	extern __shared__ __align__(16) uint32_t lds[];
	const uint32_t lane = threadIdx.x & 63u;
	const uint32_t wave = threadIdx.x >> 6;

	(void)args_by_value;
#if defined(__HIP_DEVICE_COMPILE__)
	const KArgs K = (KArgs)__builtin_amdgcn_kernarg_segment_ptr();
	auto kargs = [&]() -> KArgs {
		KArgs k = K;
		asm volatile("" : "+s"(k));
		return k;
	};
#else
	const KArgs K = &args_by_value;
	auto kargs = [&]() -> KArgs { return K; };
#endif
	DevPairScene PS = {};
	auto load_pair_boxes = [&]() {
		if constexpr (F::pair) {
			const KArgs k = kargs();
#pragma unroll
			for (int i = 0; i < 3; ++i) {
				PS.c0min[i] = k->pair.c0min[i]; PS.c0max[i] = k->pair.c0max[i];
				PS.c1min[i] = k->pair.c1min[i]; PS.c1max[i] = k->pair.c1max[i];
			}
		}
	};
	auto load_pair_scene = [&](auto with_boxes) {
		if constexpr (F::pair) {
			if constexpr (decltype(with_boxes)::value)
				load_pair_boxes();
			const KArgs k = kargs();
#pragma unroll
			for (int i = 0; i < 3; ++i) {
				PS.sky_c1[i] = k->pair.sky_c1[i]; PS.sky_c2[i] = k->pair.sky_c2[i];
			}
			PS.slot0 = k->pair.slot0; PS.slot1 = k->pair.slot1; PS.rank0 = k->pair.rank0; PS.rank1 = k->pair.rank1;
#pragma unroll
			for (int i = 0; i < 4; ++i) {
				PS.sphere[0][i] = k->pair.sphere[0][i]; PS.sphere[1][i] = k->pair.sphere[1][i];
				PS.lambert[0][i] = k->pair.lambert[0][i]; PS.lambert[1][i] = k->pair.lambert[1][i];
			}
			PS.inv_radius[0] = k->pair.inv_radius[0]; PS.inv_radius[1] = k->pair.inv_radius[1];
			PS.sky_param = k->pair.sky_param;
			PS.sky_tex_type = k->pair.sky_tex_type;
		}
	};
	DevPairPrimary PP = {};
	auto load_pair_primary = [&]() {
		if constexpr (F::pair) {
			const KArgs k = kargs();
#pragma unroll
			for (int i = 0; i < 3; ++i) {
				PP.box[0][0][i] = k->primary.box[0][0][i]; PP.box[0][1][i] = k->primary.box[0][1][i];
				PP.box[1][0][i] = k->primary.box[1][0][i]; PP.box[1][1][i] = k->primary.box[1][1][i];
			}
#pragma unroll
			for (int i = 0; i < 4; ++i) {
				PP.sphere[0][i] = k->primary.sphere[0][i]; PP.sphere[1][i] = k->primary.sphere[1][i];
			}
			PP.valid = k->primary.valid;
		}
	};
	const DevScene S_global = K->S;
	const DevRenderParams P = K->P;
	uint32_t *const stack_ovf = K->stack_ovf;
	DevScene S = S_global;

	SkyTables T;
	uint32_t sky_words = 0;
	if (SKY_LDS) {
		const uint32_t n_rows = S.sky.res_y * (S.sky.res_x + 1u);
		const uint32_t n_all = n_rows + S.sky.res_y + 1u;
		float *lds_sky = reinterpret_cast<float *>(lds);
		for (uint32_t i = threadIdx.x; i < n_all; i += blockDim.x)
			lds_sky[i] = S.sky.row_cdf[i];
		__syncthreads();
		sky_words = (n_all + 3u) & ~3u;
		const uint32_t guide_words = (S.sky.res_y + 1u) * S.sky.guide_k / 4u;
		uint32_t *lds_guide = lds + sky_words;
		const uint32_t *src_guide = reinterpret_cast<const uint32_t *>(S.sky.guide);
		for (uint32_t i = threadIdx.x; i < guide_words; i += blockDim.x)
			lds_guide[i] = src_guide[i];
		__syncthreads();
		T.row_cdf = lds_sky;
		T.marginal_cdf = lds_sky + n_rows;
		T.guide = reinterpret_cast<const uint8_t *>(lds_guide);
		sky_words += guide_words;
	} else {
		T.row_cdf = S.sky.row_cdf;
		T.marginal_cdf = S.sky.marginal_cdf;
		T.guide = S.sky.guide;
	}
	T.guide_k = S.sky.guide_k;
	T.inv_res = reinterpret_cast<KWords>(&K->S.sky.inv_res_ok);
	uint32_t blob_words = 0;
	if (!FINE && P.scene_in_lds) {
		uint32_t *lds_blob = lds + sky_words;
		blob_words = S.blob_bytes / 4u;
		for (uint32_t i = threadIdx.x; i < blob_words; i += blockDim.x)
			lds_blob[i] = S.blob[i];
		__syncthreads();
		const char *b = reinterpret_cast<const char *>(lds_blob);
		S.nodes = reinterpret_cast<const DevNode *>(b + S.off_nodes);
		S.prims = reinterpret_cast<const DevPrim *>(b + S.off_prims);
		S.shade = reinterpret_cast<const DevShade *>(b + S.off_shade);
		S.prim_rank = reinterpret_cast<const uint32_t *>(b + S.off_rank);
		S.materials = reinterpret_cast<const DevMaterial *>(b + S.off_materials);
		S.textures = reinterpret_cast<const DevTexture *>(b + S.off_textures);
		S.lights = reinterpret_cast<const uint32_t *>(b + S.off_lights);
		S.big_leaves = reinterpret_cast<const uint2 *>(b + S.off_big_leaves);
	}
	StackMem SM;
	SM.cap = P.stack_cap;
	SM.ovf_depth = P.stack_ovf_depth;
	SM.ovf = stack_ovf;
	SM.region = lds + sky_words + blob_words;
	uint32_t *stk = SM.region + wave * (P.stack_cap * kStackStride) + lane;
	uint32_t *pool = nullptr;
	if constexpr (XCHG) {
		pool = lds + (((uint32_t)(SM.region - lds) + (blockDim.x >> 6) * (P.stack_cap * kStackStride) + 3u) & ~3u);
		if (FINE) {
			if (threadIdx.x < kXchgFineHdr)
				pool[threadIdx.x] = threadIdx.x == 3u ? kXchgShaderWaves : (threadIdx.x == 4u ? (blockDim.x >> 6) - kXchgShaderWaves : 0u);
		} else if (threadIdx.x < 4u) {
			pool[threadIdx.x] = 0u;
		}
		__syncthreads();
	}

#ifdef RT_STATS
	unsigned long long st_iters[2] = {0, 0}, st_active[2] = {0, 0}, st_gen = 0, st_hist[8] = {};
	unsigned long long st_sect[16] = {}, st_mark = wall_clock64();
	unsigned long long st_fine_clock[PH_COUNT + 1] = {};
	unsigned long long st_fine_iters[PH_COUNT] = {}, st_fine_active[PH_COUNT] = {};
#endif
	const bool sky_samplable = sky_can_sample(S);
	constexpr bool kWholeItems = F::pair && !FINE;
	static_assert(!(kWholeItems && XCHG), "the exchange's records carry chunk_begin and chunk_end, not chunk_c: no whole-pixel items there");
	constexpr int known_path = F::known_materials ? kMatLambertian : kMatRead;
	constexpr bool kKeyedGen = kWholeItems && lean_gen_keys(F::pair);
	constexpr bool kItemProduct = kWholeItems && lean_gen_item_product(F::pair);

	int ph = PH_NEED_PIXEL;
	rt_rng rng = {1u, 2u, 3u, 4u};
	Ray ray;
	ray.o = ray.d = ray.inv = ray.shear = v3s(0.0f);
	uint32_t node = kRefDone;
	int sp = 0;
	float best_t = 0.0f;
	uint32_t best_prim = kNoPrim;
	bool any_hit = false;
	V3 thr = v3s(1.0f), outp = v3s(0.0f), mean = v3s(0.0f), wo = v3s(0.0f);
	Hit hit;
	hit.t = 0.0f;
	hit.point = hit.error = hit.normal = v3s(0.0f);
	hit.err_dot = 0.0f;
	hit.uvx = hit.uvy = 0.0f;
	hit.has_uv = hit.out = false;
	uint32_t mat = 0;
	uint32_t depth = 0, out_index = 0, pixel_index = 0, px = 0, py = 0;
	uint32_t sample_i = 0, chunk_begin = 0, chunk_end = P.spp, chunk_c = 0;
	uint32_t ray_count = 0;
	unsigned long long rays_total = 0;
	bool primary = true;
	uint32_t gen_hi0 = 0, gen_lo0 = 0;
	struct LightCtx {
		V3 l_wi;
		float pdf_multiplier;
		float t_limit;
		uint32_t skip;
		bool have_shadow, shadow_is_sky;
	};
	LightCtx PL;
	PL.l_wi = v3s(0.0f);
	PL.pdf_multiplier = 1.0f;
	PL.t_limit = 0.0f;
	PL.skip = kNoPrim;
	PL.have_shadow = PL.shadow_is_sky = false;

	auto begin_walk = [&](bool shadow) {
		any_hit = shadow;
		best_t = 0.0f;
		best_prim = kNoPrim;
		sp = 0;
		if (!FINE) {
			ph = PH_NODE;
			return;
		}
		if (XCHG) {
			ph = PH_WALK;
			return;
		}
		if (root_box_misses(S, ray)) {
			node = kRefDone;
			ph = shadow ? PH_SCATTER : PH_SHADE;
		} else if (S.narrow_only != 0u || !ray_is_regular(ray)) {
			ph = PH_NARROW;
		} else {
			node = S.root4_ref;
			ph = ref_is_leaf(node) ? PH_LEAF : PH_NODE;
		}
	};
	auto start_walk = [&]() {
		sp = 0;
		if (root_box_misses(S, ray)) {
			node = kRefDone;
			ph = any_hit ? PH_SCATTER : PH_SHADE;
		} else if (S.narrow_only != 0u || !ray_is_regular(ray)) {
			ph = PH_NARROW;
		} else {
			node = S.root4_ref;
			ph = ref_is_leaf(node) ? PH_LEAF : PH_NODE;
		}
	};
	auto after_step = [&]() {
		if (node == kRefDone)
			ph = any_hit ? PH_SCATTER : PH_SHADE;
		else
			ph = ref_is_leaf(node) ? PH_LEAF : PH_NODE;
	};
	auto finalize = [&](bool filter) {
		V3 c = outp;
		if (filter && (contains_nan(c) || !is_finite_any(c)))
			c = v3s(0.0f);
		if (P.sample_split > 1u) {
			mean.x += c.x;
			mean.y += c.y;
			mean.z += c.z;
		} else {
			const float i_f = (float)(sample_i + 1u);
			mean.x += (c.x - mean.x) / i_f;
			mean.y += (c.y - mean.y) / i_f;
			mean.z += (c.z - mean.z) / i_f;
		}
		rays_total += ray_count;
		sample_i += 1;
		if (sample_i == chunk_end) {
			const KArgs k = kargs();
			float *const out = k->out;
			out[3u * (size_t)out_index + 0u] = mean.x;
			out[3u * (size_t)out_index + 1u] = mean.y;
			out[3u * (size_t)out_index + 2u] = mean.z;
			ph = PH_NEED_PIXEL;
			if constexpr (kWholeItems) {
				const uint32_t log2_s = k->P.tile_log2_w >> 8;
				const uint32_t c1 = (chunk_c & (kWholePixel - 1u)) + 1u;
				if (chunk_c >= kWholePixel && (c1 >> log2_s) == 0u) {
					chunk_c += 1u;
					chunk_end = (uint32_t)(((uint64_t)(c1 + 1u) * k->P.spp) >> log2_s);
					out_index += k->P.n_work;
					mean = v3s(0.0f);
					ph = PH_GEN;
				}
			}
		} else {
			ph = PH_GEN;
		}
	};

	auto do_gen = [&]() {
		const KArgs k = kargs();
		const uint64_t seed = ((uint64_t)k->P.seed_hi << 32) | k->P.seed_lo;
		const uint64_t sample_begin = ((uint64_t)k->P.sample_begin_hi << 32) | k->P.sample_begin_lo;
		const V3 cam_o = v3(k->cam.origin[0], k->cam.origin[1], k->cam.origin[2]);
		const V3 cam_ll = v3(k->cam.lower_left[0], k->cam.lower_left[1], k->cam.lower_left[2]);
		const V3 cam_h = v3(k->cam.horizontal[0], k->cam.horizontal[1], k->cam.horizontal[2]);
		const V3 cam_v = v3(k->cam.vertical[0], k->cam.vertical[1], k->cam.vertical[2]);
		const uint32_t w1 = here_(k->P.width - 1u), h1 = here_(k->P.height - 1u);
		if constexpr (kKeyedGen) {
			uint32_t hi0 = gen_hi0, lo0 = gen_lo0;
			if constexpr (!kItemProduct)
				philox_pixel_product(pixel_index, hi0, lo0);
			rng_seed_keyed<lean_gen_keys_lead(F::pair)>(&rng, &k->gen_keys, hi0, lo0, sample_begin + chunk_begin + sample_i);
		} else {
			rt_rng_seed(&rng, seed, (uint64_t)pixel_index, sample_begin + chunk_begin + sample_i);
		}
		RT_SECTION(15);
		const float jx = rt_rng_range_f32(&rng, 0.0f, 1.0f) + (float)px, jy = rt_rng_range_f32(&rng, 0.0f, 1.0f) + (float)py;
		float u, v;
		if (here_(k->P.w1h1_ok) != 0u) {
			u = div_by_verified(jx, (float)w1, k->P.inv_w1);
			v = 1.0f - div_by_verified(jy, (float)h1, k->P.inv_h1);
		} else {
			u = div_tame_fix_(jx, (float)w1);
			v = 1.0f - div_tame_fix_(jy, (float)h1);
		}
		ray = ray_new<F>(cam_o, cam_ll + cam_h * u + cam_v * v - cam_o);
		(void)rt_rng_f32(&rng);
		thr = v3s(1.0f);
		outp = v3s(0.0f);
		depth = 0;
		ray_count = 0;
		primary = true;
		begin_walk(false);
	
	};

#ifdef RT_STATS
	unsigned long long st_lane_nodes = 0, st_lane_prims = 0, st_lane_maxsp = 0;
#endif
	auto do_node = [&]() {
#ifdef RT_STATS
		st_lane_nodes += 1;
		if ((unsigned long long)sp > st_lane_maxsp)
			st_lane_maxsp = (unsigned long long)sp;
#endif
		const bool limit_valid = any_hit ? !(PL.t_limit != PL.t_limit) : (best_prim != kNoPrim);
		if (SM.ovf_depth == 0u)
			node = descend4<PRUNE, false>(S, SM, ray, node, stk, sp, limit_valid, any_hit ? PL.t_limit : best_t);
		else
			node = descend4<PRUNE, true>(S, SM, ray, node, stk, sp, limit_valid, any_hit ? PL.t_limit : best_t);
		after_step();
	
	};

	auto do_leaf = [&]() {
		uint32_t first, count, leaf_ref;
		const bool candidate = wide_leaf_hit(S, node, ray, leaf_ref);
		leaf_range(S, leaf_ref, first, count);
		if (!candidate)
			count = 0u;
		bool occluded = false;
		for (uint32_t slot = first; slot < first + count; ++slot) {
			if (any_hit && slot == PL.skip)
				continue;
#ifdef RT_STATS
			st_lane_prims += 1;
#endif
			const PrimGeom g = load_prim<F>(S, slot);
			float t;
			if (prim_t<F>(g, ray, t) && t > 0.0f) {
				if (any_hit) {
					if (!(t >= PL.t_limit)) {
						occluded = true;
						break;
					}
				} else {
					bool take;
					if (best_prim == kNoPrim)
						take = true;
					else if (t < best_t)
						take = true;
					else if (t == best_t)
						take = S.prim_rank[slot] < S.prim_rank[best_prim];
					else
						take = false;
					if (take) {
						best_t = t;
						best_prim = slot;
					}
				}
			}
		}
		if (occluded) {
			best_prim = 0u;
			node = kRefDone;
		} else if (sp == 0) {
			node = kRefDone;
		} else {
			--sp;
			node = SM.ovf_depth == 0u ? stack_load<false>(SM, stk, sp) : stack_load<true>(SM, stk, sp);
		}
		after_step();
	
	};

	auto do_shade = [&](auto arm_tag) {
		constexpr int arm = decltype(arm_tag)::value;
		const uint32_t prim = best_prim;
		bool finish = false;
		bool filter = true;
		Hit nh;
		uint32_t nmat;
		if (prim != kNoPrim)
			make_hit<F>(S, prim, ray, best_t, nh, nmat, PS);
		else
			make_sky_hit_lean<F>(S, nh, nmat);
		const int known_new = F::known_materials ? (prim == kNoPrim ? kMatEmit : kMatLambertian) : kMatRead;

		if (METHOD == 0) {
			ray_count += 1;
			const V3 wo_n = ray.d;
// ... 490 lines not shown
		const bool is_e = (mE >> lane & 1ull) != 0ull;
		if (!will_bounce) {
			uint32_t can = nb >= kXchgMinLanes ? min(nb, slots - cB) : 0u;
			if (!fresh)
				can = min(can, cP);
			if (ph == PH_LIGHT && rB < can) {
				park_path(cB + rB);
				if (rB < cP)
					take_pixel(cP - 1u - rB);
				else
					ph = PH_NEED_PIXEL;
			}
			cB += can;
			cP -= min(can, cP);
			const uint32_t te = min(ne, cP);
			if (is_e && rE < te)
				take_pixel(cP - 1u - rE);
			cP -= te;
		} else {
			const uint32_t swaps = np >= kXchgMinLanes ? min(min(np, cB), slots - cP) : 0u;
			if (ph == PH_GEN && rP < swaps) {
				park_pixel(cP + rP);
				take_path(cB - 1u - rP);
			}
			cB -= swaps;
			cP += swaps;
			const uint32_t te = min(ne, cB);
			if (is_e && rE < te)
				take_path(cB - 1u - rE);
			cB -= te;
			if (nb == 0u && np == 0u && te == 0u) {
				const uint32_t tp = min(ne, cP);
				if (is_e && rE < tp)
					take_pixel(cP - 1u - rE);
				cP -= tp;
			}
		}
		__builtin_amdgcn_fence(__ATOMIC_RELEASE, "workgroup");
		if (lane == 0u) {
			pool[1] = cB;
			pool[2] = cP;
			__hip_atomic_store(&pool[0], 0u, __ATOMIC_RELEASE, __HIP_MEMORY_SCOPE_WORKGROUP);
		}
	};

	uint32_t wq_next = 0, wq_end = 0;
	uint32_t wq_xy = 0, wq_pbase = 0;
	auto acquire_coarse = [&]() {
		const unsigned long long need = __ballot(ph == PH_NEED_PIXEL);
		if (kAcquireBatch > 1u && (uint32_t)__popcll(need) < kAcquireBatch && __ballot(ph == PH_GEN || ph == PH_LIGHT) != 0ull)
			return;
		const KArgs k = kargs();
		const bool tiled = P.tile_log2_w != 0xFFFFFFFFu;
		uint32_t avail = 0, old_next = 0, old_xy = 0, old_pbase = 0, base = 0, log2_w = 0, log2_s = 0;
		if (need != 0ull) {
			const uint32_t n = (uint32_t)__popcll(need);
#if defined(RT_STATS) && !defined(RT_STATS_NO_HIST)
			if (lane == 0u)
				atomicAdd(&g_hist[2][n], 1ull);
#endif
			avail = wq_end - wq_next;
			old_next = wq_next, old_xy = wq_xy, old_pbase = wq_pbase;
			if (tiled)
				log2_w = k->P.tile_log2_w & 7u, log2_s = k->P.tile_log2_w >> 8;
			base = wq_end;
			if (avail < n) {
				const int leader = __ffsll((long long)need) - 1;
				uint32_t claimed = 0;
				if ((int)lane == leader)
					claimed = atomicAdd(k->work_counter, kClaim);
				base = (uint32_t)__builtin_amdgcn_readlane((int)claimed, leader);
				if (tiled) {
					const uint32_t b = base >> 6;
					const uint32_t whole = kWholeItems ? k->P.whole_claims : 0u;
					const bool is_whole = b < whole;
					const uint32_t bc = is_whole ? 0u : b - whole;
					const uint32_t kt = is_whole ? b : whole + (bc >> log2_s);
					const uint32_t sub = bc & ((1u << log2_s) - 1u);
					const uint32_t tile = k->P.shard_index + kt * k->P.shard_count;
					const uint32_t ty = tile / k->P.tiles_x;
					const uint32_t tx = tile - ty * k->P.tiles_x;
					wq_xy = (tx << log2_w) | ((ty * k->P.tile_h) << 16);
					wq_pbase = ((kt << 6) + (sub << (6u - log2_s))) | (is_whole ? kWholeClaim : 0u);
				}
				wq_next = base + (n - avail);
				wq_end = base + kClaim;
			} else {
				wq_next += n;
			}
		}
		if (ph == PH_NEED_PIXEL) {
			const uint32_t r = (uint32_t)__popcll(need & ((1ull << lane) - 1ull));
			const bool from_old = r < avail;
			const uint32_t w = from_old ? old_next + r : base + (r - avail);
			const uint32_t spp = k->P.spp;
			bool inside;
			if (tiled) {
				const uint32_t xy = from_old ? old_xy : wq_xy;
				const uint32_t in = w & 63u;
				const uint32_t pbase = from_old ? old_pbase : wq_pbase;
				const bool whole = kWholeItems && pbase >= kWholeClaim;
				const uint32_t ls = whole ? 0u : log2_s;
				const uint32_t wp = (kWholeItems ? pbase & (kWholeClaim - 1u) : pbase) + (in >> ls);
				const uint32_t c = in & ((1u << ls) - 1u);
				const uint32_t in_tile = wp & 63u;
				px = (xy & 0xFFFFu) + (in_tile & ((1u << log2_w) - 1u));
				py = (xy >> 16) + (in_tile >> log2_w);
				inside = px < k->P.width && py < k->P.height;
				pixel_index = py * k->P.width + px;
				const uint32_t first = (uint32_t)(((uint64_t)c * spp) >> log2_s);
				const uint32_t end = (uint32_t)(((uint64_t)(c + 1u) * spp) >> log2_s);
				if constexpr (kWholeItems) {
					sample_i = first;
					chunk_end = end;
					chunk_c = c | (whole ? kWholePixel : 0u);
				} else {
					chunk_begin = first;
					chunk_end = end - first;
				}
				out_index = log2_s != 0u ? c * k->P.n_work + wp : (k->P.shard_layout ? wp : pixel_index);
			} else {
				const uint32_t split = k->P.sample_split, n_work = k->P.n_work;
				inside = work_to_pixel(P, split > 1u ? w % n_work : w, px, py);
				pixel_index = py * k->P.width + px;
				if constexpr (kWholeItems)
					chunk_c = 0u;
				if (split > 1u) {
					const uint32_t c = w / n_work;
					const uint32_t first = (uint32_t)(((uint64_t)c * spp) / split);
					const uint32_t end = (uint32_t)(((uint64_t)(c + 1u) * spp) / split);
					if constexpr (kWholeItems) {
						sample_i = first;
						chunk_end = end;
					} else {
						chunk_begin = first;
						chunk_end = end - first;
					}
					out_index = w;
				} else {
					if constexpr (kWholeItems)
						sample_i = 0u;
					else
						chunk_begin = 0u;
					chunk_end = spp;
					out_index = k->P.shard_layout ? w : pixel_index;
				}
			}
			if constexpr (kItemProduct)
				philox_pixel_product(pixel_index, gen_hi0, gen_lo0);
			if (w >= k->P.n_items) {
				ph = PH_DONE;
			} else if (inside) {
				if constexpr (!kWholeItems)
					sample_i = 0;
				mean = v3s(0.0f);
				ph = PH_GEN;
			}
		}
	};
	auto acquire = [&]() {
	if constexpr (!FINE) {
		acquire_coarse();
		return;
	}
	{
		const unsigned long long need = __ballot(ph == PH_NEED_PIXEL);
		if (need != 0ull) {
			const KArgs k = kargs();
			const DevRenderParams P = k->P;
			const uint32_t n = (uint32_t)__popcll(need);
			const uint32_t avail = wq_end - wq_next;
			uint32_t base = wq_end;
			if (avail < n) {
				const int leader = __ffsll((long long)need) - 1;
				uint32_t claimed = 0;
				if ((int)lane == leader)
					claimed = atomicAdd(k->work_counter, kClaim);
				base = __shfl(claimed, leader);
			}
			if (ph == PH_NEED_PIXEL) {
				const uint32_t r = (uint32_t)__popcll(need & ((1ull << lane) - 1ull));
				const uint32_t w = r < avail ? wq_next + r : base + (r - avail);
				if (w >= P.n_items) {
					ph = PH_DONE;
				} else if (work_to_pixel(P, P.sample_split > 1u ? w % P.n_work : w, px, py)) {
					pixel_index = py * P.width + px;
					if (P.sample_split > 1u) {
						const uint32_t c = w / P.n_work;
						chunk_begin = (uint32_t)(((uint64_t)c * P.spp) / P.sample_split);
						chunk_end = (uint32_t)(((uint64_t)(c + 1u) * P.spp) / P.sample_split) - chunk_begin;
						out_index = w;
					} else {
						out_index = P.shard_layout ? w : pixel_index;
					}
					sample_i = 0;
					mean = v3s(0.0f);
					ph = PH_GEN;
				}
// ... 29 lines not shown
				if (k != PH_NODE && run < 0 && cnt[k] >= (k == PH_NARROW ? 1u : (k == PH_LEAF ? kDrainLanes : kDrainLanesHeavy))) {
					run = k;
					best_n = cnt[k];
				}
			}
			if (run < 0 && cnt[PH_NODE] > 0u && !(XCHG && xchg_shader)) {
				run = PH_NODE;
				best_n = cnt[PH_NODE];
			}
			if (run < 0) {
#pragma unroll
				for (int k = 0; k < PH_COUNT; ++k) {
					if (cnt[k] >= best_n && cnt[k] > 0u) {
						best_n = cnt[k];
						run = k;
					}
				}
			}
			if (run < 0) {
				if (XCHG && __ballot(ph == PH_WALK) != 0ull) {
					__builtin_amdgcn_s_sleep(4);
					continue;
				}
				if (__ballot(ph == PH_NEED_PIXEL) == 0ull) {
					if (XCHG && !xchg_try_exit()) {
						__builtin_amdgcn_s_sleep(4);
						continue;
					}
					break;
				}
				continue;
			}
#ifdef RT_STATS
			if (lane == 0u) {
				st_fine_iters[run] += 1;
				st_fine_active[run] += best_n;
			}
#endif
#ifdef RT_STATS
			if (lane == 0u) {
				const unsigned long long now_ = wall_clock64();
				st_fine_clock[PH_COUNT] += now_ - st_mark;
				st_mark = now_;
			}
#endif
			if (run == PH_NODE) {
#pragma unroll 1
				for (int step = 0; step < kNodeStepsPerVote; ++step)
					if (ph == PH_NODE)
						do_node();
			} else if (run == PH_LEAF) {
				if (ph == PH_LEAF)
					do_leaf();
			} else if (run == PH_GEN) {
				if (ph == PH_GEN)
					do_gen();
			} else if (run == PH_SHADE) {
				if (ph == PH_SHADE)
					do_shade(std::integral_constant<int, 0>{});
			} else if (run == PH_LIGHT) {
				if (ph == PH_LIGHT)
					do_light(PL, ray);
			} else if (run == PH_NARROW) {
				if (ph == PH_NARROW)
					do_narrow();
			} else {
				if (ph == PH_SCATTER)
					do_scatter(PL, ray);
			}
#ifdef RT_STATS
			if (lane == 0u) {
				const unsigned long long now_ = wall_clock64();
				st_fine_clock[run] += now_ - st_mark;
				st_mark = now_;
			}
#endif
		}
	}

	if constexpr (!FINE) {
		bool alive = true;
		uint32_t waited = 0;
		while (alive) {
			if (XCHG && METHOD == 1)
				exchange();
			acquire();
			const uint32_t n_light = (uint32_t)__popcll(__ballot(ph == PH_LIGHT));
			const uint32_t n_trace = (METHOD == 1 && RT_PQ_SPLIT) ? (uint32_t)__popcll(__ballot(ph == PH_GEN))
			                                                      : (uint32_t)__popcll(__ballot(ph == PH_GEN || ph == PH_NODE || ph == PH_LEAF || ph == PH_SHADE));
			constexpr bool kBodyAlways = RT_BODY_ALWAYS(KernelShape<F>::spheres_only);
			if (kBodyAlways) {
				alive = (n_light + n_trace != 0u) || __ballot(ph == PH_NEED_PIXEL) != 0ull;
				if (XCHG && METHOD == 1 && !alive)
					alive = __hip_atomic_load(&pool[1], __ATOMIC_RELAXED, __HIP_MEMORY_SCOPE_WORKGROUP) != 0u ||
					        __hip_atomic_load(&pool[2], __ATOMIC_RELAXED, __HIP_MEMORY_SCOPE_WORKGROUP) != 0u;
			}
			if (kBodyAlways || n_light + n_trace != 0u) {
				const bool run_light = (METHOD == 1) && (n_light >= kLightPhaseThreshold || n_trace == 0u || (kStarveLimit != 0u && waited >= kStarveLimit));
				waited = run_light ? 0u : waited + n_light;
	#ifdef RT_STATS
				if (lane == 0u) {
					if (!run_light) {
						st_iters[0] += 1; st_active[0] += n_trace;
						st_hist[((n_trace ? n_trace : 1u) - 1u) >> 3] += 1;
#ifndef RT_STATS_NO_HIST
						atomicAdd(&g_hist[0][n_trace], 1ull);
						atomicAdd(&g_hist[1][n_light], 1ull);
#endif
						st_gen += (unsigned long long)__popcll(__ballot(ph == PH_GEN));
					} else {
						st_iters[1] += 1; st_active[1] += n_light;
#ifndef RT_STATS_NO_HIST
						atomicAdd(&g_hist[3][n_light], 1ull);
#endif
					}
				}
	#endif
				RT_SECTION(0);
				constexpr bool kFuseRegions = METHOD == 1 && RT_PQ_SPLIT && RT_FUSE_REGIONS(KernelShape<F>::spheres_only);
				bool run_q = run_light;
				if (!run_light) {
					if (kFuseRegions) {
						if (ph == PH_GEN) {
							load_pair_scene(std::false_type{});
							do_gen();
							load_pair_primary();
							RT_SECTION(1);
							walk_closest_primary();
							RT_SECTION(2);
							do_shade(std::integral_constant<int, 1>{});
						}
						RT_SECTION(3);
						const uint32_t n_light_now = (uint32_t)__popcll(__ballot(ph == PH_LIGHT));
						run_q = n_light_now >= kLightPhaseThreshold;
						if (run_q)
							waited = 0u;
	#ifdef RT_STATS
						if (run_q && lane == 0u) {
							st_iters[1] += 1; st_active[1] += n_light_now;
						}
	#endif
					} else {
						load_pair_scene(std::true_type{});
						if (ph == PH_GEN)
							do_gen();
						RT_SECTION(1);
						walk_closest_pending();
						RT_SECTION(2);
						if (ph == PH_SHADE)
							do_shade(std::integral_constant<int, (METHOD == 1 && RT_PQ_SPLIT) ? 1 : 0>{});
						RT_SECTION(3);
					}
				}
				if (run_q) {
					LightCtx L;
					L.l_wi = v3s(0.0f);
					L.pdf_multiplier = 1.0f;
					L.t_limit = 0.0f;
					L.skip = kNoPrim;
					L.have_shadow = L.shadow_is_sky = false;
					Ray sray;
					sray.o = sray.d = sray.inv = sray.shear = v3s(0.0f);
					if (kFuseRegions) {
						if (ph == PH_LIGHT) {
							load_pair_scene(std::true_type{});
							do_light(L, sray);
							RT_SECTION(4);
							walk_shadow_pending(L, sray);
							RT_SECTION(5);
							do_scatter(L, sray);
							RT_SECTION(6);
							if (ph == PH_NODE) {
								walk_closest_pending();
								RT_SECTION(7);
								do_shade(std::integral_constant<int, 2>{});
							}
						}
						RT_SECTION(8);
					} else {
						load_pair_scene(std::true_type{});
						if (ph == PH_LIGHT)
							do_light(L, sray);
						RT_SECTION(4);
						walk_shadow_pending(L, sray);
						RT_SECTION(5);
						if (ph == PH_SCATTER)
							do_scatter(L, sray);
						RT_SECTION(6);
	#if RT_PQ_SPLIT
						walk_closest_pending();
						RT_SECTION(7);
						if (ph == PH_SHADE)
							do_shade(std::integral_constant<int, 2>{});
						RT_SECTION(8);
	#endif
					}
				}
	#if RT_PQ_SPLIT
				if (METHOD == 1) {
					ray.o = ray.d = ray.inv = ray.shear = v3s(0.0f);
					best_t = 0.0f;
					best_prim = kNoPrim;
					node = kRefDone;
					sp = 0;
					any_hit = false;
				}
	#endif
			} else {
				alive = __ballot(ph == PH_NEED_PIXEL) != 0ull;
				if (XCHG && METHOD == 1)
					alive = alive || __hip_atomic_load(&pool[1], __ATOMIC_RELAXED, __HIP_MEMORY_SCOPE_WORKGROUP) != 0u ||
					        __hip_atomic_load(&pool[2], __ATOMIC_RELAXED, __HIP_MEMORY_SCOPE_WORKGROUP) != 0u;
			}
		}
	}
#ifdef RT_STATS
	atomicAdd(&g_stats[20], st_lane_nodes);
	atomicAdd(&g_stats[21], st_lane_prims);
	atomicMax(&g_stats[22], st_lane_maxsp);
	if (lane == 0u) {
		for (int k = 0; k < 9; ++k)
			atomicAdd(&g_stats[40 + k], st_sect[k]);
		if (!FINE)
			for (int k = 9; k < 16; ++k)
				atomicAdd(&g_stats[40 + k], st_sect[k]);
		for (int k = 0; k < 8; ++k)
			atomicAdd(&g_stats[24 + k], st_hist[k]);
		for (int k = 0; k <= PH_COUNT; ++k)
			atomicAdd(&g_stats[50 + k], st_fine_clock[k]);
		atomicAdd(&g_stats[0], st_iters[0]); atomicAdd(&g_stats[1], st_active[0]);
		atomicAdd(&g_stats[2], st_iters[1]); atomicAdd(&g_stats[3], st_active[1]);
		atomicAdd(&g_stats[4], st_gen);
		for (int k = 0; k < PH_COUNT; ++k) {
			atomicAdd(&g_stats[5 + k], st_fine_iters[k]);
			atomicAdd(&g_stats[5 + PH_COUNT + k], st_fine_active[k]);
		}
	}
#endif
	unsigned long long *const rays_shot = K->rays_shot;
	if (rays_shot != nullptr) {
		for (int off = 32; off > 0; off >>= 1)
			rays_total += __shfl_down(rays_total, off);
		if (lane == 0u)
			atomicAdd(rays_shot, rays_total);
	}
}

__global__ __launch_bounds__(256) void combine_chunks_kernel(const DevRenderParams P, const float *__restrict__ partial, float *__restrict__ out)
{
	const uint32_t wp = blockIdx.x * blockDim.x + threadIdx.x;
	if (wp >= P.n_work)
		return;
	uint32_t x, y;
	if (!work_to_pixel(P, wp, x, y))
		return;
	V3 acc = v3s(0.0f);
	for (uint32_t c = 0; c < P.sample_split; ++c) {
		const float *m = partial + 3u * ((size_t)c * P.n_work + wp);
		acc.x = acc.x + m[0];
		acc.y = acc.y + m[1];
		acc.z = acc.z + m[2];
	}
	const size_t o = P.shard_layout ? (size_t)wp : (size_t)y * P.width + x;
	out[3u * o + 0u] = acc.x / (float)P.spp;
	out[3u * o + 1u] = acc.y / (float)P.spp;
	out[3u * o + 2u] = acc.z / (float)P.spp;
}

__global__ __launch_bounds__(256) void reset_kernel(uint32_t *__restrict__ work_counter, unsigned long long *__restrict__ rays_shot,
                                                    float *__restrict__ out, size_t n_out_floats)
{
	const size_t i = (size_t)blockIdx.x * blockDim.x + threadIdx.x;
	if (i == 0) {
		*work_counter = 0u;
		if (rays_shot)
			*rays_shot = 0ull;
	}
	for (size_t k = i; k < n_out_floats; k += (size_t)gridDim.x * blockDim.x)
		out[k] = 0.0f;
}
hipError_t launch_reset(hipStream_t stream, uint32_t *work_counter, unsigned long long *rays_shot, float *out, size_t n_out_floats)
{
	size_t blocks = (n_out_floats + 255) / 256;
	if (blocks < 1)
		blocks = 1;
	if (blocks > 4096)
		blocks = 4096;
	hipLaunchKernelGGL(reset_kernel, dim3((uint32_t)blocks), dim3(256), 0, stream, work_counter, rays_shot, out, n_out_floats);
	return hipGetLastError();
}

__global__ __launch_bounds__(256) void quantise_kernel(const float *__restrict__ rgb, size_t n_values, float inv_gamma, uint8_t *__restrict__ out)
{
	const size_t stride = (size_t)gridDim.x * blockDim.x;
	const size_t n4 = n_values / 4;
	for (size_t i = (size_t)blockIdx.x * blockDim.x + threadIdx.x; i < n4; i += stride) {
		const float4 v = reinterpret_cast<const float4 *>(rgb)[i];
		const uint32_t q = (uint32_t)rt_quantise_u8(v.x, inv_gamma) | ((uint32_t)rt_quantise_u8(v.y, inv_gamma) << 8) |
		                   ((uint32_t)rt_quantise_u8(v.z, inv_gamma) << 16) | ((uint32_t)rt_quantise_u8(v.w, inv_gamma) << 24);
		reinterpret_cast<uint32_t *>(out)[i] = q;
	}
	if (blockIdx.x == 0 && threadIdx.x < (n_values & 3))
		out[n4 * 4 + threadIdx.x] = rt_quantise_u8(rgb[n4 * 4 + threadIdx.x], inv_gamma);
}
__global__ __launch_bounds__(256) void quantise_unaligned_kernel(const float *__restrict__ rgb, size_t n_values, float inv_gamma, uint8_t *__restrict__ out)
{
	const size_t stride = (size_t)gridDim.x * blockDim.x;
	for (size_t i = (size_t)blockIdx.x * blockDim.x + threadIdx.x; i < n_values; i += stride)
		out[i] = rt_quantise_u8(rgb[i], inv_gamma);
}
hipError_t launch_quantise(hipStream_t stream, const float *rgb, size_t n_values, float inv_gamma, uint8_t *out)
{
	if ((reinterpret_cast<uintptr_t>(rgb) & 15u) != 0u || (reinterpret_cast<uintptr_t>(out) & 3u) != 0u) {
		size_t blocks = (n_values + 255) / 256;
		blocks = blocks < 1 ? 1 : (blocks > 16384 ? 16384 : blocks);
// ... 124 lines not shown
using FeatSimple = Feat<true, true, false, false>;

template <class F> static render_fn pick_render_f(int method, bool prune, bool fine, bool sky_lds, bool xchg)
{
#ifdef RT_ONLY_HEADLINE
	if constexpr (!(F::cmat || F::ctex))
		if (method == 1 && !prune && !fine && sky_lds && !xchg)
			return render_kernel<1, false, false, true, F>;
#ifdef RT_HEADLINE_RUNNABLE
	if constexpr (!(F::cmat || F::ctex))
		if (method == 1 && !prune && !fine && !sky_lds && !xchg)
			return render_kernel<1, false, false, false, F>;
#endif
	return nullptr;
#else
	if constexpr (F::pair) {
		if (xchg || prune || fine)
			return nullptr;
		if (method == 0)
			return render_kernel<0, false, false, false, F>;
		return sky_lds ? render_kernel<1, false, false, true, F> : render_kernel<1, false, false, false, F>;
	} else {
	if (xchg) {
		if (method == 1 && !prune && !fine)
			return sky_lds ? render_kernel<1, false, false, true, F, true> : render_kernel<1, false, false, false, F, true>;
		if (fine && method == 0)
			return render_kernel<0, true, true, false, F, true>;
		if (fine && method == 1)
			return sky_lds ? render_kernel<1, true, true, true, F, true> : render_kernel<1, true, true, false, F, true>;
		return nullptr;
	}
#define RT_PICK(M, P, G, L) \
	if (method == M && prune == P && fine == G && sky_lds == L) \
		return render_kernel<M, P, G, L, F>;
	RT_PICK(0, false, false, false)
	RT_PICK(0, true, false, false)
	RT_PICK(0, true, true, false)
	RT_PICK(1, false, false, false)
	RT_PICK(1, false, false, true)
	RT_PICK(1, true, false, false)
	RT_PICK(1, true, false, true)
	RT_PICK(1, true, true, false)
	RT_PICK(1, true, true, true)
#undef RT_PICK
	return nullptr;
	}
#endif
}

static render_fn pick_render(int method, bool prune, bool fine, bool sky_lds, int feature_set, bool xchg = false)
{
	if (method == 0)
		sky_lds = false;
	if (fine)
		prune = true;
	if (feature_set == 0)
		return pick_render_f<FeatSpheres>(method, prune, fine, sky_lds, xchg);
	if (feature_set == 1)
		return pick_render_f<FeatSimple>(method, prune, fine, sky_lds, xchg);
	if (feature_set == 3)
		return pick_render_f<FeatPair>(method, prune, fine, sky_lds, xchg);
	return pick_render_f<FeatFull>(method, prune, fine, sky_lds, xchg);
}
bool render_exchange_available(int method, bool prune, bool fine, int feature_set) { (void)feature_set; return fine || (method == 1 && !prune); }
size_t render_exchange_lds_bytes(uint32_t slots) { return (size_t)(4u + 4u + (kXchgBStride + kXchgPStride) * slots) * sizeof(uint32_t); }
uint32_t render_exchange_max_slots() { return kXchgMaxSlots; }
size_t render_exchange_fine_lds_bytes(uint32_t waves_per_block) { return (size_t)(4u + kXchgFineHdr + waves_per_block * 64u + 2u * kXchgFineSlots * kXchgRecWords) * sizeof(uint32_t); }

hipError_t render_occupancy(int method, bool prune, bool fine, bool sky_lds, int feature_set, size_t lds_bytes, int *blocks_per_cu, bool xchg,
                            uint32_t block_threads)
{
	render_fn fn = pick_render(method, prune, fine, sky_lds, feature_set, xchg);
	if (!fn)
		return hipErrorInvalidValue;
	hipError_t e = hipFuncSetAttribute(reinterpret_cast<const void *>(fn), hipFuncAttributeMaxDynamicSharedMemorySize, (int)lds_bytes);
	if (e != hipSuccess)
		return e;
	return hipOccupancyMaxActiveBlocksPerMultiprocessor(blocks_per_cu, fn, block_threads ? block_threads : render_block_threads(feature_set, fine, xchg), lds_bytes);
}

hipError_t launch_render(int method, bool prune, bool fine, bool sky_lds, int feature_set, uint32_t n_blocks, size_t lds_bytes, hipStream_t stream,
                         const DevScene &S, const DevCamera &cam, const DevRenderParams &P, float *out,
                         unsigned long long *rays_shot, uint32_t *work_counter, uint32_t *stack_ovf, bool xchg, const DevPairScene *pair,
                         const DevPairPrimary *primary, uint32_t block_threads)
{
	render_fn fn = pick_render(method, prune, fine, sky_lds, feature_set, xchg);
	if (!fn)
		return hipErrorInvalidValue;
	RenderArgs A;
	A.S = S;
	A.cam = cam;
	A.P = P;
	A.out = out;
	A.rays_shot = rays_shot;
	A.work_counter = work_counter;
	A.stack_ovf = stack_ovf;
	A.pair = pair ? *pair : DevPairScene{};
	A.primary = primary ? *primary : DevPairPrimary{};
	philox_round_keys(((uint64_t)P.seed_hi << 32) | P.seed_lo, A.gen_keys);
	hipLaunchKernelGGL(fn, dim3(n_blocks), dim3(block_threads ? block_threads : render_block_threads(feature_set, fine, xchg)), lds_bytes, stream, A);
	return hipGetLastError();
}

}
```

### raytracing-rust_amd/csrc/rt_selftest.h

```cpp
#pragma once

#include <hip/hip_runtime.h>

#include "../../include/rt_hip.h"
#include "rt_types.h"

namespace rt {

hipError_t launch_selftest_lean(hipStream_t stream, uint32_t blocks, uint64_t n_per_thread, uint64_t seed, unsigned long long *mismatches);
hipError_t launch_selftest_pair_primary(hipStream_t stream, const DevPairScene &pair, const float root_min[3], const float root_max[3], const float origin[3],
                                        const DevPairPrimary &host_block, unsigned long long *mismatches);

struct DevSkySelftest {
	uint64_t seed;
	uint64_t n;
	float *out_dirs;
	float *out_pdf_s;
	const float *dirs;
	uint64_t m;
	float *out_pdf;
};

size_t sky_selftest_lds_bytes(const DevScene &S);
hipError_t launch_sky_selftest(bool tables_in_lds, hipStream_t stream, const DevScene &S, const DevSkySelftest &P);



constexpr uint32_t kShortFormsRcpExponentCount = 8;
struct DevShortForms {
	unsigned long long *tested;
	unsigned long long *mismatches;
	unsigned long long *first_index;
	unsigned long long *sqrt_raw;
	unsigned long long *site_tested;
	unsigned long long *site_mismatches;
};
uint32_t short_forms_input_bits(int form, uint64_t index);
uint32_t short_forms_in_use();
hipError_t launch_short_forms(hipStream_t stream, const DevShortForms &D, const float *operands, uint64_t n_operands);

enum { kDivCountTested = 0, kDivCountBad = 1, kDivCountFirst = 1 + RT_DIV_FORMS, kDivCountSiteTested = 1 + 2 * RT_DIV_FORMS, kDivCountSiteInDomain,
       kDivCountSiteBad, kDivCounts = kDivCountSiteBad + RT_DIV_SITES };
struct DevDivForms {
	const uint32_t *denominators;
	uint32_t n_denominators, first_denominator;
	const int32_t *exponents;
	uint32_t n_exponent_pairs;
	unsigned long long *counts;
};
uint32_t div_forms_in_use();
hipError_t launch_div_forms(hipStream_t stream, const DevDivForms &D);
hipError_t launch_div_sites(hipStream_t stream, const float *operand_pairs, uint64_t n_pairs, unsigned long long *counts);
hipError_t launch_sky_pdf_forms(hipStream_t stream, const DevScene &S, const float *dirs, uint64_t m, float *out_pair, float *out_default);

uint32_t frame_forms_in_use();
hipError_t launch_frame_forms(hipStream_t stream, const float *vectors, uint64_t n_vectors, unsigned long long *counts);

uint32_t gen_keys_in_use();
hipError_t launch_gen_keys(hipStream_t stream, uint64_t seed, const uint32_t *cases, uint64_t n_cases, unsigned long long *counts);

hipError_t launch_pair_shadow(hipStream_t stream, const float *cases, uint64_t n_cases, unsigned long long *counts);
hipError_t launch_pair_shadow_walk(hipStream_t stream, const float *cases, uint64_t n_cases, unsigned long long *counts);

}
```

### raytracing-rust_amd/csrc/rt_selftest_forms.hip

```cpp
#include "rt_shade.h"
#include "rt_gen_keys.h"
#include "rt_selftest.h"
#include "rt_selftest_dev.h"

namespace rt {

__host__ __device__ inline uint32_t short_forms_rcp_input(uint64_t index)
{
	static_assert(kShortFormsRcpExponentCount == 8, "one case per exponent");
	int e = 0;
	switch ((uint32_t)(index >> 24)) {
	case 0: e = -81; break;
	case 1: e = -60; break;
	case 2: e = -24; break;
	case 3: e = -1; break;
	case 4: e = 0; break;
	case 5: e = 1; break;
	case 6: e = 24; break;
	default: e = 41; break;
	}
	return ((uint32_t)(index >> 23) & 1u) << 31 | (uint32_t)(127 + e) << 23 | ((uint32_t)index & 0x007FFFFFu);
}

using FormTally = Tally<RT_SHORT_FORMS>;
// ... 64 lines not shown
		T.add(RT_SHORT_SITE_RAY_NEW_PAIR, ray_new_differs<FeatPair>(dir));
		T.add(RT_SHORT_SITE_RAY_NEW_FULL, ray_new_differs<FeatFull>(dir));
		tested.add(0);
	});
	tested.flush(D.site_tested);
	T.flush(D.site_mismatches);
}

__global__ __launch_bounds__(256) void pair_shadow_kernel(const float *__restrict__ cases, uint64_t n_cases, unsigned long long *counts)
{
	Tally<RT_PAIR_SHADOW_COUNTS> T;
	for_each_case(n_cases, [&](uint64_t i) {
		const float *c = cases + i * RT_PAIR_SHADOW_CASE_FLOATS;
		const V3 center = v3(c[0], c[1], c[2]);
		const float radius = c[3];
		Ray r;
		r.o = v3(c[4], c[5], c[6]);
		r.d = v3(c[7], c[8], c[9]);
		r.inv = r.shear = v3s(0.0f);
		float t;
		const bool want = sphere_t(center, radius, r, t) && t > 0.0f;
		T.add(RT_PAIR_SHADOW_MISMATCHES, sphere_occludes_unlimited(center, radius, r) != want);
		T.add(RT_PAIR_SHADOW_ASKED_MISMATCHES, sphere_occludes_asked(center, radius, r) != want);
		T.add(RT_PAIR_SHADOW_ASKED, sphere_shadow_signs(center, radius, r).ask);
		T.add(RT_PAIR_SHADOW_TESTED);
	});
	T.flush(counts);
}
hipError_t launch_pair_shadow(hipStream_t stream, const float *cases, uint64_t n_cases, unsigned long long *counts)
{
	return launch_cases(pair_shadow_kernel, stream, n_cases, 2048u, cases, n_cases, counts);
}

struct FeatPairFullShadow : FeatPair {
	static constexpr bool sky_shadows_only = false;
};
constexpr uint32_t kWalkSlot0 = 7u, kWalkSlot1 = 3u;
__global__ __launch_bounds__(256) void pair_shadow_walk_kernel(const float *__restrict__ cases, uint64_t n_cases, unsigned long long *counts)
{
	Tally<RT_PAIR_SHADOW_WALK_COUNTS> T;
	const DevScene S = {};
	const StackMem M = {};
	for_each_case(n_cases, [&](uint64_t i) {
		const float *c = cases + i * RT_PAIR_SHADOW_WALK_CASE_FLOATS;
		DevPairScene ps = {};
		for (int k = 0; k < 4; ++k) {
			ps.sphere[0][k] = c[k];
			ps.sphere[1][k] = c[4 + k];
		}
		for (int k = 0; k < 3; ++k) {
			ps.c0min[k] = c[k] - fabsf(c[3]); ps.c0max[k] = c[k] + fabsf(c[3]);
			ps.c1min[k] = c[4 + k] - fabsf(c[7]); ps.c1max[k] = c[4 + k] + fabsf(c[7]);
		}
		ps.slot0 = kWalkSlot0;
		ps.slot1 = kWalkSlot1;
		const uint32_t skip = c[14] == 1.0f ? kWalkSlot0 : (c[14] == 2.0f ? kWalkSlot1 : kNoPrim);
		Ray r;
		r.o = v3(c[8], c[9], c[10]);
		r.d = v3(c[11], c[12], c[13]);
		r.d = r.d / mag(r.d);
		r.inv = v3(1.0f / r.d.x, 1.0f / r.d.y, 1.0f / r.d.z);
		r.shear = v3s(0.0f);
		const float no_limit = __uint_as_float(0x7FC00000u);
		const bool got = trace_any<FeatPair, false>(S, S, M, r, nullptr, no_limit, skip, ps);
		const bool want = trace_any<FeatPairFullShadow, false>(S, S, M, r, nullptr, no_limit, skip, ps);
		T.add(RT_PAIR_SHADOW_WALK_MISMATCHES, got != want);
		float tb;
		const bool c0 = aabb_does_int(ps.c0min, ps.c0max, r, tb) && ps.slot0 != skip, c1 = aabb_does_int(ps.c1min, ps.c1max, r, tb) && ps.slot1 != skip;
		const ShadowSigns s0 = sphere_shadow_signs(v3(c[0], c[1], c[2]), c[3], r), s1 = sphere_shadow_signs(v3(c[4], c[5], c[6]), c[7], r);
		const bool occ0 = c0 && s0.occluded, ask0 = c0 && s0.ask;
		const bool occ1 = !occ0 && c1 && s1.occluded, ask1 = !occ0 && c1 && s1.ask;
		T.add(RT_PAIR_SHADOW_WALK_ASKED, ask0 || ask1);
		T.add(RT_PAIR_SHADOW_WALK_ASKED_BOTH, ask0 && ask1);
		T.add(RT_PAIR_SHADOW_WALK_ASKED_WITH_OCCLUDED, (ask0 || ask1) && (occ0 || occ1));
		T.add(RT_PAIR_SHADOW_WALK_TESTED);
	});
	T.flush(counts);
}
hipError_t launch_pair_shadow_walk(hipStream_t stream, const float *cases, uint64_t n_cases, unsigned long long *counts)
{
	return launch_cases(pair_shadow_walk_kernel, stream, n_cases, 2048u, cases, n_cases, counts);
}

constexpr uint32_t kDivChunkBits = 10, kDivChunkShift = 23u - kDivChunkBits;
__host__ __device__ inline uint64_t div_forms_items(const DevDivForms &D) { return ((uint64_t)D.n_exponent_pairs * D.n_denominators) << kDivChunkShift; }
__global__ __launch_bounds__(256) void div_forms_kernel(DevDivForms D)
{
	Tally<RT_DIV_FORMS> T;
	Tally<1> tested;
	const uint32_t chunk_shift = kDivChunkShift;
	for_each_case(div_forms_items(D), [&](uint64_t item) {
		const uint64_t pair_index = item >> chunk_shift;
		const uint32_t chunk = (uint32_t)item & ((1u << chunk_shift) - 1u);
		const uint32_t e = (uint32_t)(pair_index / D.n_denominators), j = (uint32_t)(pair_index - (uint64_t)e * D.n_denominators);
		const uint32_t d_sig = (D.denominators ? D.denominators[j] : D.first_denominator + j) & 0x007FFFFFu;
		const uint32_t n_high = (uint32_t)(127 + D.exponents[2u * e]) << 23;
		const float d = __uint_as_float((uint32_t)(127 + D.exponents[2u * e + 1u]) << 23 | d_sig);
		const float r1 = lean_rcp_refined(d);
		for (uint32_t k = 0; k < (1u << kDivChunkBits); ++k) {
			const uint32_t n_sig = chunk << kDivChunkBits | k;
			const float n = __uint_as_float(n_high | n_sig);
			const float want = n / d;
			const unsigned long long index = pair_index << 23 | n_sig;
			T.note(RT_DIV_FORM_ONE_PAIR, !same_f32(lean_div_core_gfx950(n, d, r1), want), index);
			T.note(RT_DIV_FORM_TWO_PAIRS, !same_f32(lean_div_core(n, d, r1), want), index);
		}
		tested.add(0, 1ull << kDivChunkBits);
	});
	tested.flush(D.counts + kDivCountTested);
	T.flush(D.counts + kDivCountBad, D.counts + kDivCountFirst);
}
hipError_t launch_div_forms(hipStream_t stream, const DevDivForms &D) { return launch_cases(div_forms_kernel, stream, div_forms_items(D), 4096u, D); }
constexpr uint32_t div_form_bit(LeanDivForm f) { return 1u << (f == LeanDivForm::one_pair ? RT_DIV_FORM_ONE_PAIR : RT_DIV_FORM_TWO_PAIRS); }
uint32_t div_forms_in_use() { return div_form_bit(lean_div_form(true)); }

__device__ __noinline__ V3 mis_light_term_plain(V3 te, V3 le, float l_pdf, float m_pdf)
{
	const float a_sq = l_pdf * l_pdf;
	const float mis_weight = a_sq / (a_sq + m_pdf * m_pdf);
	return te * mis_weight * le / l_pdf;
}
__device__ __noinline__ V3 div3_plain(V3 v, float d) { return v / d; }
__device__ __forceinline__ bool same_v3(V3 a, V3 b) { return same_f32(a.x, b.x) && same_f32(a.y, b.y) && same_f32(a.z, b.z); }
__device__ __forceinline__ bool div_fix_domain(float n, float d)
{
	const float an = fabsf(n), ad = fabsf(d);
	const bool d_tame = ad >= 0x1p-81f && ad <= 0x1p41f;
	const bool n_tame = an >= 0x1p-81f && an <= 0x1p41f;
	const int apart = (int)(__float_as_uint(an) >> 23) - (int)(__float_as_uint(ad) >> 23);
	return d_tame && ((n_tame && apart < 96 && apart > -96) || an == 0.0f || an == INFINITY || n != n);
}
__global__ __launch_bounds__(256) void div_sites_kernel(const float *__restrict__ pairs, uint64_t n_pairs, unsigned long long *counts)
{
	Tally<kDivCounts> T;
	for_each_case(n_pairs, [&](uint64_t i) {
		const float n = pairs[2u * i], d = pairs[2u * i + 1u];
		if (div_fix_domain(n, d)) {
			T.add(kDivCountSiteInDomain);
			T.add(kDivCountSiteBad + RT_DIV_SITE_FIX, !same_f32(lean_div_fix_for<true>(n, d), n / d));
			const V3 v = v3(n, 0.0f, -INFINITY);
			T.add(kDivCountSiteBad + RT_DIV_SITE_DIV3_FIX, !same_v3(lean_div3_fix_for<true>(v, d), div3_plain(v, d)));
		}
		const V3 one = v3s(1.0f), te = v3(1.0f, 0.75f, -0.5f);
		bool ok = same_v3(mis_light_term_short(te, one, d, n), mis_light_term_plain(te, one, d, n));
		ok = ok && same_v3(mis_light_term_short(te, one, n, d), mis_light_term_plain(te, one, n, d));
		const V3 tx = v3(2.0f * n, 0.75f, -0.5f), tz = v3(0.75f, -0.5f, 2.0f * n), ta = v3s(2.0f * n);
		ok = ok && same_v3(mis_light_term_short(tx, one, 1.0f, 1.0f), mis_light_term_plain(tx, one, 1.0f, 1.0f));
		ok = ok && same_v3(mis_light_term_short(tz, one, d, d), mis_light_term_plain(tz, one, d, d));
		ok = ok && same_v3(mis_light_term_short(ta, v3(1.0f, d, -1.0f), 1.0f, 1.0f), mis_light_term_plain(ta, v3(1.0f, d, -1.0f), 1.0f, 1.0f));
		T.add(kDivCountSiteBad + RT_DIV_SITE_MIS_LIGHT_TERM, !ok);
		T.add(kDivCountSiteBad + RT_DIV_SITE_ATAN2,
		      !(same_f32(lean_atan2_for<true>(n, d), lean_atan2(n, d)) && same_f32(lean_atan2_for<true>(d, n), lean_atan2(d, n)) &&
		        same_f32(lean_atan2_for<true>(-n, d), rt_atan2f(-n, d))));
		T.add(kDivCountSiteTested);
	});
	T.flush(counts);
}
hipError_t launch_div_sites(hipStream_t stream, const float *operand_pairs, uint64_t n_pairs, unsigned long long *counts)
{
	return launch_cases(div_sites_kernel, stream, n_pairs, 2048u, operand_pairs, n_pairs, counts);
}

struct SkyPdfFormsArgs {
	DevScene S;
	const float *dirs;
	uint64_t m;
// ... 152 lines not shown
```

### raytracing-rust_amd/hip_backend.py

```python
import ctypes as C
import os
import sys

import numpy as np

from . import abi

_HERE = os.path.dirname(os.path.abspath(__file__))
LIB_PATH = os.environ.get("RT_HIP_LIB") or os.path.join(_HERE, "librt_hip.so")
_LIB = None


class RtHipError(RuntimeError):
    def __init__(self, code, message):
        super().__init__(f"rt_hip error {code}: {message}")
        self.code = code


def lib():
    global _LIB
    if _LIB is None:
        if not os.path.exists(LIB_PATH):
            raise RtHipError(abi.RT_ERR_NO_DEVICE, f"{LIB_PATH} not built (run `make -C raytracing-rust_amd/csrc`); "
                             "the HIP back end has no CPU fallback")
# ... 135 lines not shown
    return int(lib().rt_device_count())


def selftest_lean(device=0, n_per_thread=64, seed=1):
    out = (C.c_uint64 * 9)()
    _check(lib().rt_selftest_lean(C.c_int(device), C.c_uint64(n_per_thread), C.c_uint64(seed), out))
    return [int(x) for x in out]


def selftest_short_forms(device=0, operands=None):
    res = abi.ShortFormsResult()
    if operands is None:
        _check(lib().rt_selftest_short_forms(C.c_int(device), None, C.c_uint64(0), C.byref(res)))
        forms = {name: (int(f.tested), int(f.mismatches), int(f.first_mismatch) if f.mismatches else None)
                 for name, f in zip(abi.SHORT_FORM_NAMES, res.form)}
        raw = {k: int(getattr(res, "sqrt_raw_" + k)) for k in ("exact", "high", "low", "other")}
        return {"forms": forms, "sqrt_raw": raw, "in_use": _in_use(abi.SHORT_FORM_NAMES, res.in_use)}
    ops = np.ascontiguousarray(operands, dtype=np.float32).ravel()
    _check(lib().rt_selftest_short_forms(C.c_int(device), _p(ops, C.c_float), C.c_uint64(ops.size), C.byref(res)))
    return {"sites": dict(zip(abi.SHORT_SITE_NAMES, (int(x) for x in res.site_mismatches))), "tested": int(res.site_tested)}


def selftest_div_forms(denominators=None, exponents=((0, 0),), first_denominator=0, n_denominators=None, operands=None, device=0):
    res = abi.DivFormsResult()
    if operands is not None:
        ops = np.ascontiguousarray(operands, dtype=np.float32)
        if ops.ndim != 2 or ops.shape[1] != 2:
            raise ValueError(f"operands must be (n, 2), got {ops.shape}")
        _check(lib().rt_selftest_div_forms(C.c_int(device), None, _p(ops, C.c_float), C.c_uint64(ops.shape[0]), C.byref(res)))
        return {"tested": int(res.site_tested), "in_domain": int(res.site_in_domain),
                "sites": dict(zip(abi.DIV_SITE_NAMES, (int(x) for x in res.site_mismatches)))}
    exps = np.ascontiguousarray(exponents, dtype=np.int32).reshape(-1, 2)
    sl = abi.DivFormsSlice()
    sl.exponents, sl.n_exponent_pairs = _p(exps, C.c_int32), exps.shape[0]
    if denominators is not None:
        dens = np.ascontiguousarray(denominators, dtype=np.uint32).ravel()
        sl.denominators, sl.n_denominators = _p(dens, C.c_uint32), dens.size
    else:
        sl.denominators, sl.n_denominators, sl.first_denominator = None, int(n_denominators), int(first_denominator)
    _check(lib().rt_selftest_div_forms(C.c_int(device), C.byref(sl), None, C.c_uint64(0), C.byref(res)))
    forms = {name: (int(res.mismatches[k]), (int(res.first_numerator[k]), int(res.first_denominator[k])) if res.mismatches[k] else None)
             for k, name in enumerate(abi.DIV_FORM_NAMES)}
    return {"tested": int(res.tested), "forms": forms, "in_use": _in_use(abi.DIV_FORM_NAMES, res.in_use)}


def selftest_sky_pdf_forms(scene, dirs):
    dirs = np.ascontiguousarray(dirs, dtype=np.float32)
    if dirs.ndim != 2 or dirs.shape[1] != 3:
        raise ValueError(f"dirs must be (m, 3), got {dirs.shape}")
    a, b = np.empty(dirs.shape[0], dtype=np.float32), np.empty(dirs.shape[0], dtype=np.float32)
    _check(lib().rt_selftest_sky_pdf_forms(scene._h, _p(dirs, C.c_float), C.c_uint64(dirs.shape[0]), _p(a, C.c_float), _p(b, C.c_float)))
    return a, b


def selftest_frame_forms(vectors, device=0):
    return _selftest_cases("frame_forms", vectors, device)


def philox_round_keys(seed):
    keys = np.zeros((10, 2), dtype=np.uint32)
    lib().rt_philox_round_keys.restype = None
    lib().rt_philox_round_keys(C.c_uint64(seed & 0xFFFFFFFFFFFFFFFF), _p(keys, C.c_uint32))
    return keys


def selftest_gen_keys(seed, cases, device=0):
    return _selftest_cases("gen_keys", cases, device, C.c_uint64(seed & 0xFFFFFFFFFFFFFFFF))


def selftest_pair_shadow(cases, device=0):
    return _selftest_cases("pair_shadow", cases, device)


def selftest_pair_shadow_walk(cases, device=0):
    return _selftest_cases("pair_shadow_walk", cases, device)


def selftest_pair_primary(scene, origin):
    valid, bad = C.c_uint32(), C.c_uint64()
    _check(lib().rt_selftest_pair_primary(scene._h, _f3(origin), C.byref(valid), C.byref(bad)))
    return bool(valid.value), int(bad.value)


def camera_new(origin, lookat, vup, fov, aspect_ratio, aperture, focus_dist):
    cam = abi.Camera()
    _check(lib().rt_camera_new(C.byref(cam), _f3(origin), _f3(lookat), _f3(vup), C.c_float(fov),
                               C.c_float(aspect_ratio), C.c_float(aperture), C.c_float(focus_dist)))
    return cam


HIT_DTYPE = np.dtype([("t", "<f4"), ("point", "<f4", 3), ("error", "<f4", 3), ("normal", "<f4", 3), ("uv", "<f4", 2),
                      ("has_uv", "<i4"), ("out", "<i4"), ("material", "<u4"), ("found", "<u4"), ("index", "<u8")])
NODE_DTYPE = np.dtype([("min", "<f4", 3), ("max", "<f4", 3), ("children", "<i8", 2), ("primitive_offset", "<u8"),
                       ("number_primitives", "<u8")])


WIDE_NODE_DTYPE = np.dtype([("origin", "<f4", 3), ("exps", "<u4"), ("qlo", "<u4", 3), ("qhi", "<u4", 3), ("child", "<u4", 4),
                            ("pad", "<u4", 2)])


def _pack_rays(origins, directions):
    o = np.asarray(origins, dtype=np.float32).reshape(-1, 3)
    d = np.asarray(directions, dtype=np.float32).reshape(-1, 3)
    return np.ascontiguousarray(np.concatenate([o, d], axis=1))


class HipScene:

    def __init__(self, scene_description, device=0, devices=None):
        self._desc = scene_description.desc()
        self._h = C.c_void_p()
        if devices is not None:
            devices = [int(d) for d in devices]
            self.device = devices[0]
            self.devices = devices
            arr = (C.c_int * len(devices))(*devices)
            _check(lib().rt_scene_create_multi(C.byref(self._desc), arr, C.c_uint32(len(devices)), C.byref(self._h)))
        else:
            self.device = device
            self.devices = [device]
            _check(lib().rt_scene_create(C.byref(self._desc), C.c_int(device), C.byref(self._h)))

    def device_count(self):
        n = C.c_uint32()
        _check(lib().rt_scene_device_count(self._h, C.byref(n)))
        return n.value

    def close(self):
        if self._h:
            lib().rt_scene_destroy(self._h)
            self._h = C.c_void_p()

    def __del__(self):
        try:
            self.close()
        except Exception:
            pass

    def counts(self):
        a, b, c = C.c_uint64(), C.c_uint64(), C.c_uint64()
        _check(lib().rt_scene_counts(self._h, C.byref(a), C.byref(b), C.byref(c)))
        return a.value, b.value, c.value

    def nodes(self):
        n = self.counts()[0]
        out = np.zeros(max(1, n), dtype=NODE_DTYPE)
        _check(lib().rt_scene_get_nodes(self._h, out.ctypes.data_as(C.POINTER(abi.BvhNode)), C.c_uint64(n)))
        return out[:n]

    def primitive_order(self):
        n = self.counts()[1]
        out = np.zeros(max(1, n), dtype=np.uint64)
        _check(lib().rt_scene_get_primitive_order(self._h, _p(out, C.c_uint64), C.c_uint64(n)))
        return out[:n]

    def lights(self):
        n = self.counts()[2]
        out = np.zeros(max(1, n), dtype=np.uint64)
        _check(lib().rt_scene_get_lights(self._h, _p(out, C.c_uint64), C.c_uint64(n)))
        return out[:n]

    def wide_tree(self):
        n, root, depth = C.c_uint64(), C.c_uint32(), C.c_uint32()
        _check(lib().rt_scene_wide_info(self._h, C.byref(n), C.byref(root), C.byref(depth)))
        nodes = np.zeros(max(1, n.value), dtype=WIDE_NODE_DTYPE)
        boxes = np.zeros((max(1, self.counts()[1]), 8), dtype=np.float32)
# ... 700 lines not shown
```

Baseline: 41440.

## Add conservative sky-tile classification and a fast sky-only sample loop

Before rendering, the host computes a conservative cone test for each pixel against the scene's two pair spheres, with error margins and neighbour-pixel padding. At claim time a wave ballots whether every lane's tile provably sees only sky and, if so, tags the claim. When all active lanes hold sky-tagged items, the wave runs a dedicated loop that generates the camera direction and evaluates sky emission without BVH traversal. This removes intersection work for background pixels, but adds per-claim test cost, extra kernel state and code size, and relies on the margin analysis staying conservative.

```diff
diff --git a/include/rt_hip.h b/include/rt_hip.h
--- a/include/rt_hip.h
+++ b/include/rt_hip.h
@@ -218,7 +218,8 @@
 
 int rt_scene_set_traversal(rt_scene *scene, int mode);
 typedef enum rt_tuning_key { RT_TUNE_TRAVERSAL = 0, RT_TUNE_FEATURE_SET = 1, RT_TUNE_SCENE_IN_LDS = 2, RT_TUNE_SCHEDULE = 3, RT_TUNE_WALK = 4,
-                             RT_TUNE_STACK_CAP = 5, RT_TUNE_EXCHANGE = 6, RT_TUNE_WHOLE_PIXEL_SHARE = 7, RT_TUNE_RADIANCE_GROUPS = 8 } rt_tuning_key;
+                             RT_TUNE_STACK_CAP = 5, RT_TUNE_EXCHANGE = 6, RT_TUNE_WHOLE_PIXEL_SHARE = 7, RT_TUNE_RADIANCE_GROUPS = 8,
+                             RT_TUNE_SKY_RUN = 10 } rt_tuning_key;
 int rt_scene_set_tuning(rt_scene *scene, int key, int value);
 int rt_plan_work_items(const rt_render_opts *opts, uint32_t split, int share, uint64_t resident_waves, uint32_t *whole_claims,
                        uint64_t *n_items);
@@ -260,7 +261,9 @@
 	uint32_t sample_split;
 	uint32_t whole_claims;
 	uint64_t n_items;
-	char kernel[160];
+	uint32_t sky_run;
+	uint32_t reserved;
+	char kernel[152];
 } rt_launch_info;
 int rt_last_launch_info(const rt_scene *scene, rt_launch_info *out);
 
@@ -653,6 +656,8 @@
 
 int rt_selftest_pair_primary(rt_scene *scene, const float origin[3], uint32_t *valid, uint64_t *mismatches);
 
+int rt_selftest_sky_tiles(rt_scene *scene, const rt_camera *camera, const rt_render_opts *opts, uint8_t *out_flags, uint64_t n_tiles);
+
 int rt_selftest_sky(rt_scene *scene, int tables_in_lds, uint64_t seed, uint64_t n, float *out_dirs, float *out_pdf_of_sample,
                     const float *dirs, uint64_t m, float *out_pdf);
 
diff --git a/raytracing-rust_amd/abi.py b/raytracing-rust_amd/abi.py
--- a/raytracing-rust_amd/abi.py
+++ b/raytracing-rust_amd/abi.py
@@ -18,6 +18,7 @@
 RT_LAYOUT_FRAME, RT_LAYOUT_SHARD = range(2)
 RT_TUNE_TRAVERSAL, RT_TUNE_FEATURE_SET, RT_TUNE_SCENE_IN_LDS, RT_TUNE_SCHEDULE, RT_TUNE_WALK, RT_TUNE_STACK_CAP, RT_TUNE_EXCHANGE, RT_TUNE_WHOLE_PIXEL_SHARE = range(8)
 RT_TUNE_RADIANCE_GROUPS = 8
+RT_TUNE_SKY_RUN = 10
 
 NO_INDEX = 0xFFFFFFFFFFFFFFFF
 RT_DEVICE_NONE = -1
@@ -187,7 +188,9 @@
         ("sample_split", C.c_uint32),
         ("whole_claims", C.c_uint32),
         ("n_items", C.c_uint64),
-        ("kernel", C.c_char * 160),
+        ("sky_run", C.c_uint32),
+        ("reserved", C.c_uint32),
+        ("kernel", C.c_char * 152),
     ]
 
 
@@ -691,6 +694,7 @@
     "rt_selftest_pair_shadow",
     "rt_selftest_pair_shadow_walk",
     "rt_selftest_pair_primary",
+    "rt_selftest_sky_tiles",
     "rt_selftest_sky",
     "rt_render_aov",
     "rt_render_aov_device",
diff --git a/raytracing-rust_amd/csrc/rt_api.cpp b/raytracing-rust_amd/csrc/rt_api.cpp
--- a/raytracing-rust_amd/csrc/rt_api.cpp
+++ b/raytracing-rust_amd/csrc/rt_api.cpp
@@ -673,6 +673,11 @@
 			return fail(RT_ERR_INVALID_ARGUMENT, "radiance groups must be 0 (automatic) or 1..65536 workgroups");
 		s->radiance_groups = (uint32_t)value;
 		return RT_OK;
+	case RT_TUNE_SKY_RUN:
+		if (value < -1 || value > 1)
+			return fail(RT_ERR_INVALID_ARGUMENT, "sky run must be -1 (automatic), 0 (off) or 1 (on where the kernel has it)");
+		s->sky_run = value;
+		return RT_OK;
 	default:
 		return fail(RT_ERR_INVALID_ARGUMENT, "unknown tuning key");
 	}
@@ -966,7 +971,7 @@
 	P.scene_in_lds = scene_lds ? 1u : 0u;
 	bool sky_lds = false;
 	const int feature_set =
-	    (s->feature_set == 0 && s->pair_tree && !s->feature_set_forced && !prune && !fine && s->exchange_mode != 1) ? 3 : s->feature_set;
+	    (s->feature_set == 0 && s->pair_tree && !s->feature_set_forced && !prune && !fine && s->exchange_mode != 1 && g.n_work < kPairMaxWork) ? 3 : s->feature_set;
 	bool xchg = s->exchange_mode == 1 && render_exchange_available(o->render_method, prune, fine, feature_set);
 	const bool xchg_fine = xchg && fine;
 	uint32_t block_threads = render_block_threads(feature_set, fine, xchg_fine);
@@ -1369,14 +1374,17 @@
 		HIP_TRY(launch_reset(stream, s->d_work_counter, reinterpret_cast<unsigned long long *>(d_rays_shot), d_out_rgb, zero_floats));
 	}
 	fill_launch_info(plan, o, s->n_cus, &s->last_launch);
+	const bool sky_run = sky_run_applies(s, plan.feature_set, g.n_work, P.tile_log2_w != 0xFFFFFFFFu);
+	s->last_launch.sky_run = sky_run ? 1u : 0u;
 	const DevCamera cam = dev_camera(camera);
 	DevPairPrimary primary{};
 	if (plan.feature_set == 3)
 		pair_primary_terms(s->pair, plan.dev.root_min, plan.dev.root_max, v3(cam.origin[0], cam.origin[1], cam.origin[2]), primary);
+	const DevSkyTiles sky_tiles = sky_tiles_block(s, primary, cam, (uint32_t)o->width, (uint32_t)o->height, sky_run);
 	HIP_TRY(hipEventRecord(s->ev_start, stream));
 	HIP_TRY(launch_render(o->render_method, plan.prune, plan.fine, plan.sky_lds, plan.feature_set, plan.n_blocks, plan.lds_bytes, stream, plan.dev, cam, P,
 	                      render_target, reinterpret_cast<unsigned long long *>(d_rays_shot), s->d_work_counter, s->d_stack_ovf, plan.xchg,
-	                      plan.feature_set == 3 ? &s->pair : nullptr, plan.feature_set == 3 ? &primary : nullptr, plan.block_threads));
+	                      plan.feature_set == 3 ? &s->pair : nullptr, plan.feature_set == 3 ? &primary : nullptr, plan.block_threads, sky_tiles));
 	HIP_TRY(hipEventRecord(s->ev_stop, stream));
 	if (plan.split > 1u)
 		HIP_TRY(launch_combine(stream, P, s->d_partial, d_out_rgb));
diff --git a/raytracing-rust_amd/csrc/rt_api_internal.h b/raytracing-rust_amd/csrc/rt_api_internal.h
--- a/raytracing-rust_amd/csrc/rt_api_internal.h
+++ b/raytracing-rust_amd/csrc/rt_api_internal.h
@@ -10,6 +10,7 @@
 #include "rt_build.h"
 #include "rt_layout.h"
 #include "rt_types.h"
+#include "rt_sky_tiles.h"
 
 extern thread_local std::string g_error;
 
@@ -74,6 +75,7 @@
 	int exchange_mode = 0;
 	int whole_share = kWholeShareDefault;
 	uint32_t radiance_groups = 0;
+	int sky_run = -1;
 	uint32_t stack_depth_narrow = 2;
 	uint32_t *d_stack_ovf = nullptr;
 	size_t stack_ovf_words = 0;
@@ -175,6 +177,19 @@
 	return t;
 }
 
+constexpr uint64_t kPairMaxWork = 1ull << 30;
+inline bool sky_run_applies(const rt_scene *s, int feature_set, uint64_t n_work, bool tiled)
+{
+	return s->sky_run != 0 && feature_set == 3 && tiled && n_work < kPairMaxWork;
+}
+inline rt::DevSkyTiles sky_tiles_block(const rt_scene *s, const rt::DevPairPrimary &primary, const rt::DevCamera &cam, uint32_t width, uint32_t height, bool applies)
+{
+	rt::DevSkyTiles t{};
+	if (applies && s->pair_tree)
+		rt::sky_tiles_terms(s->pair, primary, cam, width, height, t);
+	return t;
+}
+
 inline rt::DevCamera dev_camera(const rt_camera *camera)
 {
 	rt::DevCamera cam;
diff --git a/raytracing-rust_amd/csrc/rt_api_query.cpp b/raytracing-rust_amd/csrc/rt_api_query.cpp
--- a/raytracing-rust_amd/csrc/rt_api_query.cpp
+++ b/raytracing-rust_amd/csrc/rt_api_query.cpp
@@ -467,4 +467,33 @@
 	return RT_OK;
 }
 
-}
+int rt_selftest_sky_tiles(rt_scene *s, const rt_camera *camera, const rt_render_opts *o, uint8_t *out_flags, uint64_t n_tiles)
+{
+	if (!s || !camera || !o || !out_flags)
+		return fail(RT_ERR_INVALID_ARGUMENT, "null argument");
+	if (int rc = need_device(s); rc != RT_OK)
+		return rc;
+	if (o->width < 2 || o->height < 2 || o->width >= 65536 || o->height >= 65536)
+		return fail(RT_ERR_INVALID_ARGUMENT, "width and height must be in [2, 65536)");
+	const FrameTiling t = frame_tiling(o);
+	if (n_tiles != (uint64_t)t.tiles_x * t.tiles_y)
+		return fail(RT_ERR_INVALID_ARGUMENT, "n_tiles must be the tiles of the frame the options describe");
+	std::memset(out_flags, 0, (size_t)n_tiles);
+	uint32_t log2_w = 0;
+	while (log2_w < 7u && (1u << log2_w) != t.tile_w)
+		++log2_w;
+	if (!s->pair_tree || t.tile_w * t.tile_h != 64u || log2_w >= 7u)
+		return RT_OK;
+	const DevCamera cam = dev_camera(camera);
+	DevPairPrimary primary{};
+	pair_primary_terms(s->pair, s->dev.root_min, s->dev.root_max, v3(cam.origin[0], cam.origin[1], cam.origin[2]), primary);
+	const DevSkyTiles block = sky_tiles_block(s, primary, cam, (uint32_t)o->width, (uint32_t)o->height, true);
+	std::vector<unsigned long long> words((size_t)((n_tiles + 7u) / 8u), 0ull);
+	RT_TRY(run_cases(s->device, nullptr, 0, words.data(), words.size(), "selftest_sky_tiles", [&](unsigned long long *d, void *) {
+		return launch_sky_tiles(nullptr, block, (uint32_t)o->width, (uint32_t)o->height, log2_w, t.tiles_x, n_tiles, reinterpret_cast<uint8_t *>(d));
+	}));
+	std::memcpy(out_flags, words.data(), (size_t)n_tiles);
+	return RT_OK;
+}
+
+}
diff --git a/raytracing-rust_amd/csrc/rt_intersect.h b/raytracing-rust_amd/csrc/rt_intersect.h
--- a/raytracing-rust_amd/csrc/rt_intersect.h
+++ b/raytracing-rust_amd/csrc/rt_intersect.h
@@ -9,6 +9,20 @@
 	V3 o, d, inv, shear;
 };
 
+RT_FN bool ray_dir_is_tame(V3 direction, float m2)
+{
+	const float smallest = fmin_(fmin_(fabsf(direction.x), fabsf(direction.y)), fabsf(direction.z));
+	return smallest >= 0x1p-60f && m2 >= 0x1p-40f && m2 <= 0x1p40f;
+}
+template <class F> RT_FN V3 ray_new_dir(V3 direction)
+{
+#if defined(__HIP_DEVICE_COMPILE__) && !defined(RT_NO_LEAN)
+	const float m2 = dot(direction, direction);
+	if (__builtin_expect(ray_dir_is_tame(direction, m2), 1))
+		return lean_div3_for<lean_ray_norm_short(F::pair)>(direction, lean_sqrt(m2));
+#endif
+	return direction / mag(direction);
+}
 template <class F> __device__ __forceinline__ Ray ray_new(V3 origin, V3 direction)
 {
 	Ray r;
diff --git a/raytracing-rust_amd/csrc/rt_render.h b/raytracing-rust_amd/csrc/rt_render.h
--- a/raytracing-rust_amd/csrc/rt_render.h
+++ b/raytracing-rust_amd/csrc/rt_render.h
@@ -1,6 +1,7 @@
 #pragma once
 #include <hip/hip_runtime.h>
 #include "rt_types.h"
+#include "rt_sky_tiles.h"
 
 namespace rt {
 size_t render_lds_bytes(const DevScene &S, bool sky_lds, bool scene_lds, uint32_t waves_per_block, uint32_t stack_cap);
@@ -18,7 +19,7 @@
 hipError_t launch_render(int method, bool prune, bool fine, bool sky_lds, int feature_set, uint32_t n_blocks, size_t lds_bytes, hipStream_t stream,
                          const DevScene &S, const DevCamera &cam, const DevRenderParams &P, float *out,
                          unsigned long long *rays_shot, uint32_t *work_counter, uint32_t *stack_ovf, bool xchg, const DevPairScene *pair,
-                         const DevPairPrimary *primary, uint32_t block_threads = 0);
+                         const DevPairPrimary *primary, uint32_t block_threads, const DevSkyTiles &sky_tiles);
 hipError_t launch_combine(hipStream_t stream, const DevRenderParams &P, const float *partial, float *out);
 hipError_t launch_scatter_shard(hipStream_t stream, const DevRenderParams &P, const float *shard, float *frame);
 hipError_t launch_sum_u64(hipStream_t stream, const unsigned long long *parts, uint32_t n, unsigned long long *out);
diff --git a/raytracing-rust_amd/csrc/rt_render.hip b/raytracing-rust_amd/csrc/rt_render.hip
--- a/raytracing-rust_amd/csrc/rt_render.hip
+++ b/raytracing-rust_amd/csrc/rt_render.hip
@@ -1,5 +1,6 @@
 #include "rt_shade.h"
 #include "rt_gen_keys.h"
+#include "rt_sky_tiles.h"
 #include "rt_render.h"
 
 namespace rt {
@@ -32,6 +33,12 @@
 constexpr uint32_t kClaim = 64;
 constexpr uint32_t kWholePixel = 64u;
 constexpr uint32_t kWholeClaim = 1u << 31;
+#ifndef RT_PAIR_SKY_RUN
+#define RT_PAIR_SKY_RUN 1
+#endif
+constexpr uint32_t kSkyClaim = 1u << 30;
+constexpr uint32_t kSkyItem = 128u;
+static_assert(kSkyItem > kWholePixel && kSkyClaim < kWholeClaim, "the flags sit above the chunk number and below the whole-claim bit");
 #ifndef RT_ACQUIRE_BATCH
 #define RT_ACQUIRE_BATCH 1
 #endif
@@ -135,6 +142,7 @@
 	DevPairScene pair;
 	DevPairPrimary primary;
 	DevGenKeys gen_keys;
+	DevSkyTiles sky_tiles;
 };
 #if defined(__HIP_DEVICE_COMPILE__)
 typedef const __attribute__((address_space(4))) RenderArgs *KArgs;
@@ -287,6 +295,7 @@
 	constexpr int known_path = F::known_materials ? kMatLambertian : kMatRead;
 	constexpr bool kKeyedGen = kWholeItems && lean_gen_keys(F::pair);
 	constexpr bool kItemProduct = kWholeItems && lean_gen_item_product(F::pair);
+	constexpr bool kSkyRun = kWholeItems && RT_PAIR_SKY_RUN != 0;
 
 	int ph = PH_NEED_PIXEL;
 	rt_rng rng = {1u, 2u, 3u, 4u};
@@ -392,7 +401,7 @@
 			if constexpr (kWholeItems) {
 				const uint32_t log2_s = k->P.tile_log2_w >> 8;
 				const uint32_t c1 = (chunk_c & (kWholePixel - 1u)) + 1u;
-				if (chunk_c >= kWholePixel && (c1 >> log2_s) == 0u) {
+				if ((chunk_c & kWholePixel) != 0u && (c1 >> log2_s) == 0u) {
 					chunk_c += 1u;
 					chunk_end = (uint32_t)(((uint64_t)(c1 + 1u) * k->P.spp) >> log2_s);
 					out_index += k->P.n_work;
@@ -443,8 +452,47 @@
 	
 	};
 
+	auto gen_direction = [&]() -> V3 {
+		const KArgs k = kargs();
+		const uint64_t seed = ((uint64_t)k->P.seed_hi << 32) | k->P.seed_lo;
+		const uint64_t sample_begin = ((uint64_t)k->P.sample_begin_hi << 32) | k->P.sample_begin_lo;
+		const V3 cam_o = v3(k->cam.origin[0], k->cam.origin[1], k->cam.origin[2]);
+		const V3 cam_ll = v3(k->cam.lower_left[0], k->cam.lower_left[1], k->cam.lower_left[2]);
+		const V3 cam_h = v3(k->cam.horizontal[0], k->cam.horizontal[1], k->cam.horizontal[2]);
+		const V3 cam_v = v3(k->cam.vertical[0], k->cam.vertical[1], k->cam.vertical[2]);
+		const uint32_t w1 = here_(k->P.width - 1u), h1 = here_(k->P.height - 1u);
+		if constexpr (kKeyedGen) {
+			uint32_t hi0 = gen_hi0, lo0 = gen_lo0;
+			if constexpr (!kItemProduct)
+				philox_pixel_product(pixel_index, hi0, lo0);
+			rng_seed_keyed<lean_gen_keys_lead(F::pair)>(&rng, &k->gen_keys, hi0, lo0, sample_begin + chunk_begin + sample_i);
+		} else {
+			rt_rng_seed(&rng, seed, (uint64_t)pixel_index, sample_begin + chunk_begin + sample_i);
+		}
+		RT_SECTION(15);
+		const float jx = rt_rng_range_f32(&rng, 0.0f, 1.0f) + (float)px, jy = rt_rng_range_f32(&rng, 0.0f, 1.0f) + (float)py;
+		float u, v;
+		if (here_(k->P.w1h1_ok) != 0u) {
+			u = div_by_verified(jx, (float)w1, k->P.inv_w1);
+			v = 1.0f - div_by_verified(jy, (float)h1, k->P.inv_h1);
+		} else {
+			u = div_tame_fix_(jx, (float)w1);
+			v = 1.0f - div_tame_fix_(jy, (float)h1);
+		}
+		return cam_ll + cam_h * u + cam_v * v - cam_o;
+	};
+	auto do_sky_sample = [&]() {
+		const V3 d = ray_new_dir<F>(gen_direction());
+		Hit nh;
+		uint32_t nmat;
+		make_sky_hit_lean<F>(S, nh, nmat);
+		outp = v3s(0.0f) + emission_of_hit<F>(S, PS, nmat, true, nh, d);
+		ray_count = METHOD == 0 ? 1u : 0u;
+		finalize(METHOD == 0);
+	};
+
 #ifdef RT_STATS
-	unsigned long long st_lane_nodes = 0, st_lane_prims = 0, st_lane_maxsp = 0;
+	unsigned long long st_lane_nodes = 0, st_lane_prims = 0, st_lane_maxsp = 0, st_sky_samples = 0, st_sky_runs = 0, st_sky_clock = 0, st_allsky_clock = 0, st_allsky_iters = 0, st_iter_t0 = 0;
 #endif
 	auto do_node = [&]() {
 #ifdef RT_STATS
@@ -1101,6 +1149,20 @@
 					const uint32_t tx = tile - ty * k->P.tiles_x;
 					wq_xy = (tx << log2_w) | ((ty * k->P.tile_h) << 16);
 					wq_pbase = ((kt << 6) + (sub << (6u - log2_s))) | (is_whole ? kWholeClaim : 0u);
+					if constexpr (kSkyRun) {
+						if (k->sky_tiles.enabled != 0u) {
+							DevSkyTiles ST;
+#pragma unroll
+							for (int i = 0; i < 3; ++i) {
+								ST.base[i] = k->sky_tiles.base[i]; ST.step_x[i] = k->sky_tiles.step_x[i]; ST.step_y[i] = k->sky_tiles.step_y[i];
+								ST.n[0][i] = k->sky_tiles.n[0][i]; ST.n[1][i] = k->sky_tiles.n[1][i];
+							}
+							ST.k[0] = k->sky_tiles.k[0]; ST.k[1] = k->sky_tiles.k[1];
+							const bool sees_sky = sky_lane_passes(ST, tx << log2_w, ty * k->P.tile_h, log2_w, lane, k->P.width, k->P.height);
+							if (__ballot(!sees_sky) == 0ull)
+								wq_pbase |= kSkyClaim;
+						}
+					}
 				}
 				wq_next = base + (n - avail);
 				wq_end = base + kClaim;
@@ -1120,7 +1182,7 @@
 				const uint32_t pbase = from_old ? old_pbase : wq_pbase;
 				const bool whole = kWholeItems && pbase >= kWholeClaim;
 				const uint32_t ls = whole ? 0u : log2_s;
-				const uint32_t wp = (kWholeItems ? pbase & (kWholeClaim - 1u) : pbase) + (in >> ls);
+				const uint32_t wp = (kWholeItems ? pbase & ((kSkyRun ? kSkyClaim : kWholeClaim) - 1u) : pbase) + (in >> ls);
 				const uint32_t c = in & ((1u << ls) - 1u);
 				const uint32_t in_tile = wp & 63u;
 				px = (xy & 0xFFFFu) + (in_tile & ((1u << log2_w) - 1u));
@@ -1132,7 +1194,7 @@
 				if constexpr (kWholeItems) {
 					sample_i = first;
 					chunk_end = end;
-					chunk_c = c | (whole ? kWholePixel : 0u);
+					chunk_c = c | (whole ? kWholePixel : 0u) | ((kSkyRun && (pbase & kSkyClaim) != 0u) ? kSkyItem : 0u);
 				} else {
 					chunk_begin = first;
 					chunk_end = end - first;
@@ -1328,9 +1390,42 @@
 		bool alive = true;
 		uint32_t waited = 0;
 		while (alive) {
+#ifdef RT_STATS
+			st_iter_t0 = wall_clock64();
+#endif
 			if (XCHG && METHOD == 1)
 				exchange();
 			acquire();
+			if constexpr (kSkyRun) {
+				const unsigned long long m_gen = __ballot(ph == PH_GEN);
+				if (m_gen != 0ull && __ballot(ph < PH_NEED_PIXEL && !(ph == PH_GEN && (chunk_c & kSkyItem) != 0u)) == 0ull) {
+					const KArgs k = kargs();
+#pragma unroll
+					for (int i = 0; i < 3; ++i) {
+						PS.sky_c1[i] = k->pair.sky_c1[i]; PS.sky_c2[i] = k->pair.sky_c2[i];
+					}
+					PS.sky_param = k->pair.sky_param;
+					PS.sky_tex_type = k->pair.sky_tex_type;
+#ifdef RT_STATS
+					st_sky_runs += 1;
+					RT_SECTION(0);
+#endif
+					do {
+#ifdef RT_STATS
+						st_sky_samples += (unsigned long long)__popcll(__ballot(ph == PH_GEN));
+#endif
+						if (ph == PH_GEN)
+							do_sky_sample();
+					} while (__ballot(ph == PH_GEN) == m_gen);
+#ifdef RT_STATS
+					{
+						const unsigned long long now_ = wall_clock64();
+						st_sky_clock += now_ - st_mark;
+						st_mark = now_;
+					}
+#endif
+				}
+			}
 			const uint32_t n_light = (uint32_t)__popcll(__ballot(ph == PH_LIGHT));
 			const uint32_t n_trace = (METHOD == 1 && RT_PQ_SPLIT) ? (uint32_t)__popcll(__ballot(ph == PH_GEN))
 			                                                      : (uint32_t)__popcll(__ballot(ph == PH_GEN || ph == PH_NODE || ph == PH_LEAF || ph == PH_SHADE));
@@ -1377,6 +1472,12 @@
 							do_shade(std::integral_constant<int, 1>{});
 						}
 						RT_SECTION(3);
+#ifdef RT_STATS
+						if (n_light == 0u && n_trace != 0u && __ballot(ph == PH_LIGHT) == 0ull) {
+							st_allsky_clock += wall_clock64() - st_iter_t0;
+							st_allsky_iters += 1;
+						}
+#endif
 						const uint32_t n_light_now = (uint32_t)__popcll(__ballot(ph == PH_LIGHT));
 						run_q = n_light_now >= kLightPhaseThreshold;
 						if (run_q)
@@ -1477,6 +1578,11 @@
 		atomicAdd(&g_stats[0], st_iters[0]); atomicAdd(&g_stats[1], st_active[0]);
 		atomicAdd(&g_stats[2], st_iters[1]); atomicAdd(&g_stats[3], st_active[1]);
 		atomicAdd(&g_stats[4], st_gen);
+		atomicAdd(&g_stats[58], st_sky_samples);
+		atomicAdd(&g_stats[59], st_sky_runs);
+		atomicAdd(&g_stats[60], st_sky_clock);
+		atomicAdd(&g_stats[61], st_allsky_clock);
+		atomicAdd(&g_stats[62], st_allsky_iters);
 		for (int k = 0; k < PH_COUNT; ++k) {
 			atomicAdd(&g_stats[5 + k], st_fine_iters[k]);
 			atomicAdd(&g_stats[5 + PH_COUNT + k], st_fine_active[k]);
@@ -1767,7 +1873,7 @@
 hipError_t launch_render(int method, bool prune, bool fine, bool sky_lds, int feature_set, uint32_t n_blocks, size_t lds_bytes, hipStream_t stream,
                          const DevScene &S, const DevCamera &cam, const DevRenderParams &P, float *out,
                          unsigned long long *rays_shot, uint32_t *work_counter, uint32_t *stack_ovf, bool xchg, const DevPairScene *pair,
-                         const DevPairPrimary *primary, uint32_t block_threads)
+                         const DevPairPrimary *primary, uint32_t block_threads, const DevSkyTiles &sky_tiles)
 {
 	render_fn fn = pick_render(method, prune, fine, sky_lds, feature_set, xchg);
 	if (!fn)
@@ -1782,6 +1888,7 @@
 	A.stack_ovf = stack_ovf;
 	A.pair = pair ? *pair : DevPairScene{};
 	A.primary = primary ? *primary : DevPairPrimary{};
+	A.sky_tiles = sky_tiles;
 	philox_round_keys(((uint64_t)P.seed_hi << 32) | P.seed_lo, A.gen_keys);
 	hipLaunchKernelGGL(fn, dim3(n_blocks), dim3(block_threads ? block_threads : render_block_threads(feature_set, fine, xchg)), lds_bytes, stream, A);
 	return hipGetLastError();
diff --git a/raytracing-rust_amd/csrc/rt_selftest.h b/raytracing-rust_amd/csrc/rt_selftest.h
--- a/raytracing-rust_amd/csrc/rt_selftest.h
+++ b/raytracing-rust_amd/csrc/rt_selftest.h
@@ -4,6 +4,7 @@
 
 #include "../../include/rt_hip.h"
 #include "rt_types.h"
+#include "rt_sky_tiles.h"
 
 namespace rt {
 
@@ -62,4 +63,6 @@
 hipError_t launch_pair_shadow(hipStream_t stream, const float *cases, uint64_t n_cases, unsigned long long *counts);
 hipError_t launch_pair_shadow_walk(hipStream_t stream, const float *cases, uint64_t n_cases, unsigned long long *counts);
 
+hipError_t launch_sky_tiles(hipStream_t stream, const DevSkyTiles &T, uint32_t width, uint32_t height, uint32_t log2_w, uint32_t tiles_x, uint64_t n_tiles, uint8_t *out);
+
 }
diff --git a/raytracing-rust_amd/csrc/rt_selftest_forms.hip b/raytracing-rust_amd/csrc/rt_selftest_forms.hip
--- a/raytracing-rust_amd/csrc/rt_selftest_forms.hip
+++ b/raytracing-rust_amd/csrc/rt_selftest_forms.hip
@@ -170,6 +170,23 @@
 	return launch_cases(pair_shadow_walk_kernel, stream, n_cases, 2048u, cases, n_cases, counts);
 }
 
+__global__ __launch_bounds__(256) void sky_tile_flags_kernel(const DevSkyTiles T, uint32_t width, uint32_t height, uint32_t log2_w, uint32_t tiles_x, uint64_t n_tiles,
+                                                        uint8_t *__restrict__ out)
+{
+	const uint32_t lane = threadIdx.x & 63u;
+	for (uint64_t tile = (uint64_t)blockIdx.x * 4u + (threadIdx.x >> 6); tile < n_tiles; tile += (uint64_t)gridDim.x * 4u) {
+		const uint32_t ty = (uint32_t)(tile / tiles_x), tx = (uint32_t)(tile - (uint64_t)ty * tiles_x);
+		const bool sees_sky = sky_lane_passes(T, tx << log2_w, ty * (64u >> log2_w), log2_w, lane, width, height);
+		const unsigned long long bad = __ballot(!sees_sky);
+		if (lane == 0u)
+			out[tile] = (T.enabled != 0u && bad == 0ull) ? 1u : 0u;
+	}
+}
+hipError_t launch_sky_tiles(hipStream_t stream, const DevSkyTiles &T, uint32_t width, uint32_t height, uint32_t log2_w, uint32_t tiles_x, uint64_t n_tiles, uint8_t *out)
+{
+	return launch_cases(sky_tile_flags_kernel, stream, n_tiles * 64u, 2048u, T, width, height, log2_w, tiles_x, n_tiles, out);
+}
+
 constexpr uint32_t kDivChunkBits = 10, kDivChunkShift = 23u - kDivChunkBits;
 __host__ __device__ inline uint64_t div_forms_items(const DevDivForms &D) { return ((uint64_t)D.n_exponent_pairs * D.n_denominators) << kDivChunkShift; }
 __global__ __launch_bounds__(256) void div_forms_kernel(DevDivForms D)
diff --git a/raytracing-rust_amd/csrc/rt_sky_tiles.h b/raytracing-rust_amd/csrc/rt_sky_tiles.h
--- /dev/null
+++ b/raytracing-rust_amd/csrc/rt_sky_tiles.h
@@ -0,0 +1,118 @@
+#pragma once
+
+#include <cmath>
+
+#include "rt_types.h"
+
+namespace rt {
+
+#ifndef RT_SKY_MARGIN_RHO
+#define RT_SKY_MARGIN_RHO 2.0
+#endif
+constexpr double kSkyMarginRho = RT_SKY_MARGIN_RHO;
+
+struct alignas(64) DevSkyTiles {
+	float base[3];
+	float step_x[3];
+	float step_y[3];
+	float n[2][3];
+	float k[2];
+	uint32_t enabled;
+	uint32_t pad[14];
+};
+static_assert(sizeof(DevSkyTiles) == 128, "DevSkyTiles: two 64-byte lines");
+
+RT_FN bool sky_pixel_passes(const DevSkyTiles &t, uint32_t px, uint32_t py)
+{
+	const float fx = (float)px, fy = (float)py;
+	const V3 c = v3(t.base[0] + t.step_x[0] * fx + t.step_y[0] * fy, t.base[1] + t.step_x[1] * fx + t.step_y[1] * fy,
+	                t.base[2] + t.step_x[2] * fx + t.step_y[2] * fy);
+	const float len = sqrtf(dot(c, c));
+	const bool p0 = dot(c, v3(t.n[0][0], t.n[0][1], t.n[0][2])) < t.k[0] * len;
+	const bool p1 = dot(c, v3(t.n[1][0], t.n[1][1], t.n[1][2])) < t.k[1] * len;
+	return p0 && p1;
+}
+RT_FN bool sky_lane_passes(const DevSkyTiles &t, uint32_t x0, uint32_t y0, uint32_t log2_w, uint32_t lane, uint32_t width, uint32_t height)
+{
+	const int32_t tw = (int32_t)(1u << log2_w), th = (int32_t)(64u >> log2_w);
+	const int32_t lx = (int32_t)x0 + (int32_t)(lane & ((1u << log2_w) - 1u)), ly = (int32_t)y0 + (int32_t)(lane >> log2_w);
+	bool ok = true;
+	for (int32_t b = -1; b <= 1; ++b)
+		for (int32_t a = -1; a <= 1; ++a) {
+			const int32_t px = lx + a * tw, py = ly + b * th;
+			const bool outside = px < 0 || py < 0 || px >= (int32_t)width || py >= (int32_t)height;
+			ok = ok && (outside || sky_pixel_passes(t, (uint32_t)px, (uint32_t)py));
+		}
+	return ok;
+}
+inline bool sky_tile_passes(const DevSkyTiles &t, uint32_t x0, uint32_t y0, uint32_t log2_w, uint32_t width, uint32_t height)
+{
+	if (t.enabled == 0u)
+		return false;
+	for (uint32_t lane = 0; lane < 64u; ++lane)
+		if (!sky_lane_passes(t, x0, y0, log2_w, lane, width, height))
+			return false;
+	return true;
+}
+
+inline void sky_tiles_terms(const DevPairScene &q, const DevPairPrimary &pp, const DevCamera &cam, uint32_t width, uint32_t height, DevSkyTiles &t)
+{
+	t = DevSkyTiles{};
+	t.k[0] = t.k[1] = -2.0f;
+	if (width < 2u || height < 2u || width >= 65536u || height >= 65536u || pp.valid == 0u)
+		return;
+	const double u = 0x1p-24, pi = 3.14159265358979323846;
+	double o[3], ll[3], h[3], v[3], base[3], sx[3], sy[3];
+	for (int i = 0; i < 3; ++i) {
+		o[i] = cam.origin[i]; ll[i] = cam.lower_left[i]; h[i] = cam.horizontal[i]; v[i] = cam.vertical[i];
+		if (!std::isfinite(o[i]) || !std::isfinite(ll[i]) || !std::isfinite(h[i]) || !std::isfinite(v[i]))
+			return;
+		sx[i] = h[i] / (double)(width - 1u);
+		sy[i] = -v[i] / (double)(height - 1u);
+		base[i] = ll[i] - o[i] + h[i] * (0.5 / (double)(width - 1u)) + v[i] * (1.0 - 0.5 / (double)(height - 1u));
+	}
+	auto norm = [](const double a[3]) { return std::sqrt(a[0] * a[0] + a[1] * a[1] + a[2] * a[2]); };
+	const double nrm[3] = {h[1] * v[2] - h[2] * v[1], h[2] * v[0] - h[0] * v[2], h[0] * v[1] - h[1] * v[0]};
+	const double g0[3] = {ll[0] - o[0], ll[1] - o[1], ll[2] - o[2]};
+	const double nn = norm(nrm);
+	if (!(nn > 0.0) || !std::isfinite(nn))
+		return;
+	const double dist = std::fabs(g0[0] * nrm[0] + g0[1] * nrm[1] + g0[2] * nrm[2]) / nn;
+	const double M = norm(ll) + norm(h) + norm(v) + norm(o);
+	const double Mc = norm(base) + (double)width * norm(sx) + (double)height * norm(sy);
+	const double half_diag = 0.5 * (norm(h) / (double)(width - 1u) + norm(v) / (double)(height - 1u));
+	if (!(dist > 0.0) || !std::isfinite(dist) || !std::isfinite(M) || !std::isfinite(Mc) || !(half_diag < dist))
+		return;
+	const double rho = std::asin(half_diag / dist);
+	const double slop = 16.0 * u * (1.0 + M / dist), e_cos = 16.0 * u * (1.0 + Mc / dist);
+	if (!(slop < 1e-3) || !(e_cos < 1e-3))
+		return;
+	for (int i = 0; i < 3; ++i) {
+		t.base[i] = (float)base[i]; t.step_x[i] = (float)sx[i]; t.step_y[i] = (float)sy[i];
+		if (!std::isfinite(t.base[i]) || !std::isfinite(t.step_x[i]) || !std::isfinite(t.step_y[i]))
+			return;
+	}
+	for (int s = 0; s < 2; ++s) {
+		const double dp[3] = {pp.sphere[s][0], pp.sphere[s][1], pp.sphere[s][2]};
+		const double D = norm(dp), r = std::fabs((double)q.sphere[s][3]);
+		for (int i = 0; i < 3; ++i)
+			t.n[s][i] = D > 0.0 ? (float)(dp[i] / D) : 0.0f;
+		if (!(pp.sphere[s][3] > 0.0f) || !(r < D) || !(D >= 0x1p-40 && D <= 0x1p40) || !(r >= 0x1p-40 && r <= 0x1p40))
+			continue;
+		const double theta = std::asin(r / D);
+		double phi0 = theta + kSkyMarginRho * rho;
+		if (phi0 > pi / 2 - 1e-6)
+			phi0 = std::fmax(phi0, pi / 2 + 1e-6);
+		else if (!(std::sin(phi0) - std::sin(theta) >= 16.0 * u))
+			continue;
+		const double a = phi0 + rho + slop;
+		if (!(a < pi))
+			continue;
+		float k = (float)(std::cos(a) - e_cos);
+		k = std::nextafterf(std::nextafterf(k, -3.0f), -3.0f);
+		t.k[s] = k;
+	}
+	t.enabled = 1u;
+}
+
+}
diff --git a/raytracing-rust_amd/hip_backend.py b/raytracing-rust_amd/hip_backend.py
--- a/raytracing-rust_amd/hip_backend.py
+++ b/raytracing-rust_amd/hip_backend.py
@@ -241,6 +241,14 @@
     return bool(valid.value), int(bad.value)
 
 
+def selftest_sky_tiles(scene, camera, opts):
+    tw, th = int(opts.tile_width) or 8, int(opts.tile_height) or 8
+    tiles_x, tiles_y = (int(opts.width) + tw - 1) // tw, (int(opts.height) + th - 1) // th
+    out = np.zeros(tiles_x * tiles_y, dtype=np.uint8)
+    _check(lib().rt_selftest_sky_tiles(scene._h, C.byref(camera), C.byref(opts), _p(out, C.c_uint8), C.c_uint64(out.size)))
+    return out.reshape(tiles_y, tiles_x)
+
+
 def camera_new(origin, lookat, vup, fov, aspect_ratio, aperture, focus_dist):
     cam = abi.Camera()
     _check(lib().rt_camera_new(C.byref(cam), _f3(origin), _f3(lookat), _f3(vup), C.c_float(fov),
```

After: 43000 (median of 6 runs). 3.8% higher.
